# eudald-seeslab/mmsbm

Measured on NVIDIA B200. Metric: rating-updates/sec, higher is better.
Workload: dtype f64

## Files before the change

mmsbm_b200/build.py:

```python
import concurrent.futures as cf
import os
import subprocess
import sys

HERE = os.path.dirname(os.path.abspath(__file__))
CSRC = os.path.join(HERE, "csrc")
LIB = os.path.join(HERE, "libmmsbm_b200.so")
SOURCES = ["em_step.cu", "em_small.cu", "seg_inst_ch1.cu", "seg_inst_ch2.cu", "seg_inst_ch4.cu", "seg_inst_pair.cu", "seg_inst_hexa.cu", "graph_build.cu",
           "reductions.cu", "host_api.cu", "sharded_run.cu", "fold_in.cu"]
NVCC_FLAGS = [
    "-gencode", "arch=compute_100a,code=sm_100a", "-O3", "-lineinfo", "-std=c++17",
    "-Xcompiler", "-fPIC,-O3,-Wall", "-DMMSBM_B200",
]


def _nvcc():
    for cand in (os.environ.get("NVCC"), "/usr/local/cuda/bin/nvcc", "nvcc"):
        if cand and (os.path.isabs(cand) and os.path.exists(cand) or not os.path.isabs(cand)):
            return cand
    raise RuntimeError("nvcc not found")


def _stale(target, deps):
    if not os.path.exists(target):
        return True
    t = os.path.getmtime(target)
    return any(os.path.getmtime(d) > t for d in deps)


def build_library(force=False, verbose=False, check=False):
    nvcc = _nvcc()
    suffix, extra, lib = ("_chk.o", ["-DMMSBM_BOUNDS_CHECK"], LIB.replace(".so", "_check.so")) if check \
        else (".o", ["-DNDEBUG"], LIB)
    headers = [os.path.join(CSRC, "common.cuh"), os.path.join(CSRC, "segment_pass.cuh"), os.path.join(CSRC, "em_internal.cuh"),
               os.path.join(HERE, "..", "include", "mmsbm_b200.h"), os.path.abspath(__file__)]
    objs, jobs = [], []
    for src in SOURCES:
        s = os.path.join(CSRC, src)
        o = os.path.join(CSRC, src[:-3] + suffix)
        objs.append(o)
        if force or _stale(o, [s] + headers):
            cmd = [nvcc] + NVCC_FLAGS + extra + (["-Xptxas", "-v"] if verbose else []) + ["-c", s, "-o", o]
            jobs.append(cmd)
    if jobs:
        with cf.ThreadPoolExecutor(max_workers=len(jobs)) as ex:
            for cmd, res in zip(jobs, ex.map(lambda c: subprocess.run(c, capture_output=True, text=True), jobs)):
                if verbose or res.returncode:
                    sys.stderr.write(" ".join(cmd) + "\n" + res.stdout + res.stderr)
                if res.returncode:
                    raise RuntimeError("nvcc failed for " + cmd[-3])
    if jobs or force or _stale(lib, objs):
        cmd = [nvcc, "-shared", "-o", lib] + objs + ["-lcudart", "-ldl"]
        res = subprocess.run(cmd, capture_output=True, text=True)
        if res.returncode:
            sys.stderr.write(res.stdout + res.stderr)
            raise RuntimeError("link failed")
    return lib


if __name__ == "__main__":
    print(build_library(force="--force" in sys.argv, verbose="-v" in sys.argv, check="--check" in sys.argv))
```

mmsbm_b200/csrc/em_internal.cuh:

```cuda
#pragma once
#include "common.cuh"
#include "segment_pass.cuh"

namespace mmsbm {

constexpr int kPrSlabs = 128;

int env_int(const char* name, int dflt);
int sm_count();
void set_reserved_ctas(int n);

struct RunPlan { int hexas, pairs, pair_group0, single_from; };
RunPlan plan_runs(int NBp, int n_runs, bool hexa_table);

int launch_prep_p(const double* pr, int K, int L, int R, int ldk, int ldl, int n_runs, double* pw_u,
                  double* pn_u, double* pw_i, double* pn_i, cudaStream_t st);

int launch_interleave(const double* src, double* dst, int n_src, int n_dst, int row0, int ld,
                      int group0, int groups, int gs, cudaStream_t st);

int launch_w(const double* own, const double* pw, double* W, int M, int LD, int RNB, int n_runs,
             cudaStream_t st);
struct RowPublish {
  double* dst[3];
  int gs[3], group0[3], groups[3];
  int n_all, row0;
};
int launch_n(const double* G, const double* pn, const double* own, const int32_t* deg, double* out,
             int M, int LD, int RNB, int normalize, int n_runs, cudaStream_t st,
             const RowPublish* publish = nullptr);

int launch_segment_pass_and_fixup(SegArgs a, const double* nbr_pairs, const double* nbr_hexa,
                                  int64_t n_ratings, int n_runs, cudaStream_t st, bool no_long_segments = false);

int launch_pr(const double* own, const double* g, double* partial, const double* pr, double* pr_out,
              int nseg, int NA, int lda, int NBp, int K, int L, int R, int n_runs, bool transposed,
              bool normalize, cudaStream_t st);
int launch_finalize_pr(double* pr, int kl_total, int R, cudaStream_t st);

bool em_small_applicable(int64_t N, int R, int K, int L, int S);
size_t em_small_partial_elems(int R, int K);
int launch_em_small(const int32_t* useg, const int32_t* uadj, const int32_t* udeg, const int32_t* iseg,
                    const int32_t* iadj, const int32_t* ideg, const int32_t* usched, const int32_t* isched, int64_t N,
                    int U, int I, int R, int K, int L, int S, int iterations, double* theta_a, double* eta_a,
                    double* pr_a, double* theta_b, double* eta_b, double* pr_b, double* partial, size_t partial_elems,
                    cudaStream_t st);

}
```

mmsbm_b200/csrc/em_step.cu:

```cuda
#include <stdlib.h>

#include "common.cuh"
#include "em_internal.cuh"
#include "segment_pass.cuh"

namespace mmsbm {

constexpr int kPrThreads = 128;
constexpr int kPrBatch = 16;
constexpr int kGemmThreads = 256;
constexpr int kGemmBK = 32;
constexpr int kGemmTR = 4;

__global__ void __launch_bounds__(128) segment_fixup_kernel(const SegArgs A) {
  const int run = blockIdx.y, RNB = A.R * A.NBp;
  const int n_long = __ldg(A.sched + 2);
  const int32_t* long_seg = A.sched + 4 + 3 * A.pmax;
  const int32_t* long_slot0 = long_seg + A.lmax;
  for (int li = blockIdx.x; li < n_long; li += gridDim.x) {
    const int sg = __ldg(long_seg + li), s0 = __ldg(long_slot0 + li), s1 = __ldg(long_slot0 + li + 1);
    MMSBM_DEV_CHECK(sg >= 0 && sg < A.nseg && s0 >= 0 && s0 < s1 && s1 <= A.smax);
    const double* src = A.partial + ((size_t)run * A.smax + s0) * RNB;
    double* dst = A.wg + ((size_t)run * A.nseg + sg) * RNB;
    for (int o = threadIdx.x; o < RNB; o += blockDim.x) {
      double acc = 0.0;
      for (int k = 0; k < s1 - s0; ++k) acc += src[(size_t)k * RNB + o];
      dst[o] = acc;
    }
  }
}

__global__ void interleave_runs_kernel(const double* __restrict__ src, double* __restrict__ dst, int n_src,
                                       int n_dst, int row0, int ld, int group0, int groups, int gs) {
  const int c4 = ld >> 2;
  const size_t total = (size_t)groups * n_src * gs * c4;
  const size_t t = (size_t)blockIdx.x * blockDim.x + threadIdx.x;
  if (t >= total) return;
  const int c = (int)(t % c4);
  const int j = (int)((t / c4) % gs);
  const size_t rest = t / c4 / gs;
  const int id = (int)(rest % n_src);
  const size_t p = group0 + rest / n_src;
  const double4_t v = ldg256(src + (((size_t)(gs * p + j) * n_src + id) * ld + 4 * c));
  stg256(dst + (((p * n_dst + row0 + id) * gs + j) * ld + 4 * c), v);
}

__global__ void prep_p_kernel(const double* pr, int K, int L, int R, int ldk, int ldl, double* pw_u,
                              double* pn_u, double* pw_i, double* pn_i) {
  const int run = blockIdx.y;
  const int total = ldk * ldl * R;
  const int t = blockIdx.x * blockDim.x + threadIdx.x;
  if (t >= total) return;
  const int r = t % R, kl = t / R, lp = kl % ldl, kp = kl / ldl;
  double v = 0.0;
  if (kp < K && lp < L) v = __ldg(pr + (((size_t)run * K + kp) * L + lp) * R + r);
  const size_t base = (size_t)run * total;
  const int rnb_u = R * ldl, rnb_i = R * ldk;
  pw_u[base + (size_t)kp * rnb_u + r * ldl + lp] = v;
  pn_u[base + (size_t)(r * ldl + lp) * ldk + kp] = v;
  pw_i[base + (size_t)lp * rnb_i + r * ldk + kp] = v;
  pn_i[base + (size_t)(r * ldk + kp) * ldl + lp] = v;
}

struct GemmArgs {
  const double* A;
  const double* B;
  double* C;
  const double* own;
  const int32_t* deg;
  int M, N, Kd, lda, rg, normalize;
  int b_resident;
};

template <bool EPI>
__global__ void __launch_bounds__(kGemmThreads) small_gemm_kernel(const GemmArgs g) {
  constexpr int TR = kGemmTR;
  extern __shared__ __align__(32) unsigned char smem_raw[];
  const int BM = TR * g.rg, AS = kGemmBK + 2;
  double* Bs = reinterpret_cast<double*>(smem_raw);
  double* As = Bs + (size_t)(g.b_resident ? g.Kd : kGemmBK) * g.N;
  const int run = blockIdx.y;
  const int ncg = g.N >> 2, half = g.N >> 1;
  const int rgid = threadIdx.x / ncg, cg = threadIdx.x - rgid * ncg;
  const bool active = rgid < g.rg;
  const double* A = g.A + (size_t)run * g.M * g.lda;
  const double2* B2 = reinterpret_cast<const double2*>(g.B + (size_t)run * g.Kd * g.N);
  double2* Bs2 = reinterpret_cast<double2*>(Bs);
  if (g.b_resident)
    for (int t = threadIdx.x; t < (g.Kd * g.N) >> 1; t += kGemmThreads) Bs2[t] = __ldg(B2 + t);
  const int n_tiles = (g.M + BM - 1) / BM;
  for (int tile = blockIdx.x; tile < n_tiles; tile += gridDim.x) {
    const int row0 = tile * BM;
    double acc[TR][4];
#pragma unroll
    for (int i = 0; i < TR; ++i)
#pragma unroll
      for (int j = 0; j < 4; ++j) acc[i][j] = 0.0;

    for (int k0 = 0; k0 < g.Kd; k0 += kGemmBK) {
      const int bk = min(kGemmBK, g.Kd - k0);
      const int bk2 = bk >> 1;
      __syncthreads();
      for (int t = threadIdx.x; t < BM * bk2; t += kGemmThreads) {
        const int m = t / bk2, p2 = t - m * bk2;
        double2 v = make_double2(0.0, 0.0);
        if (row0 + m < g.M) v = __ldg(reinterpret_cast<const double2*>(A + (size_t)(row0 + m) * g.lda + k0) + p2);
        *reinterpret_cast<double2*>(As + m * AS + 2 * p2) = v;
      }
      if (!g.b_resident)
        for (int t = threadIdx.x; t < (bk * g.N) >> 1; t += kGemmThreads)
          Bs2[t] = __ldg(B2 + (((size_t)k0 * g.N) >> 1) + t);
      __syncthreads();
      if (active) {
        const double* ap = As + (size_t)(TR * rgid) * AS;
        const double* bp = Bs + (size_t)(g.b_resident ? k0 : 0) * g.N + 2 * cg;
        for (int kk = 0; kk < bk; kk += 2) {
          const double2 b00 = *reinterpret_cast<const double2*>(bp + (size_t)kk * g.N);
          const double2 b01 = *reinterpret_cast<const double2*>(bp + (size_t)kk * g.N + half);
          const double2 b10 = *reinterpret_cast<const double2*>(bp + (size_t)(kk + 1) * g.N);
          const double2 b11 = *reinterpret_cast<const double2*>(bp + (size_t)(kk + 1) * g.N + half);
#pragma unroll
          for (int i = 0; i < TR; ++i) {
            const double2 a = *reinterpret_cast<const double2*>(ap + i * AS + kk);
            acc[i][0] = fma(a.x, b00.x, acc[i][0]); acc[i][1] = fma(a.x, b00.y, acc[i][1]);
            acc[i][2] = fma(a.x, b01.x, acc[i][2]); acc[i][3] = fma(a.x, b01.y, acc[i][3]);
            acc[i][0] = fma(a.y, b10.x, acc[i][0]); acc[i][1] = fma(a.y, b10.y, acc[i][1]);
            acc[i][2] = fma(a.y, b11.x, acc[i][2]); acc[i][3] = fma(a.y, b11.y, acc[i][3]);
          }
        }
      }
    }
    if (active) {
#pragma unroll
      for (int i = 0; i < TR; ++i) {
        const int m = row0 + TR * rgid + i;
        if (m >= g.M) continue;
        const size_t off = ((size_t)run * g.M + m) * g.N + 2 * cg;
        double2 v0 = make_double2(acc[i][0], acc[i][1]), v1 = make_double2(acc[i][2], acc[i][3]);
        if (EPI) {
          const double2 o0 = __ldg(reinterpret_cast<const double2*>(g.own + off));
          const double2 o1 = __ldg(reinterpret_cast<const double2*>(g.own + off + half));
          v0.x *= o0.x; v0.y *= o0.y; v1.x *= o1.x; v1.y *= o1.y;
          if (g.normalize) {
            const double d = (double)max(__ldg(g.deg + m), 1);
            v0.x = v0.x / d; v0.y = v0.y / d; v1.x = v1.x / d; v1.y = v1.y / d;
          }
        }
        *reinterpret_cast<double2*>(g.C + off) = v0;
        *reinterpret_cast<double2*>(g.C + off + half) = v1;
      }
    }
  }
}

constexpr int kRowThreads = 256;

template <int LD, int ROWS>
__global__ void __launch_bounds__(kRowThreads) row_w_kernel(const double* __restrict__ own,
                                                            const double* __restrict__ pw,
                                                            double* __restrict__ W, int M, int RNB) {
  extern __shared__ __align__(32) unsigned char smem_raw[];
  double* Ps = reinterpret_cast<double*>(smem_raw);
  const int run = blockIdx.y;
  {
    const double2* src = reinterpret_cast<const double2*>(pw + (size_t)run * LD * RNB);
    double2* dst = reinterpret_cast<double2*>(Ps);
    for (int t = threadIdx.x; t < (LD * RNB) >> 1; t += kRowThreads) dst[t] = __ldg(src + t);
  }
  __syncthreads();
  const double* own_run = own + (size_t)run * M * LD;
  double* w_run = W + (size_t)run * M * RNB;
  for (int m0 = blockIdx.x * (kRowThreads * ROWS) + threadIdx.x; m0 < M; m0 += gridDim.x * (kRowThreads * ROWS)) {
    double o[ROWS][LD];
    int mr[ROWS];
#pragma unroll
    for (int j = 0; j < ROWS; ++j) {
      mr[j] = m0 + j * kRowThreads;
      const int mc = mr[j] < M ? mr[j] : m0;
#pragma unroll
      for (int c = 0; c < LD / 4; ++c) {
        const double4_t v = ldg256(own_run + (size_t)mc * LD + 4 * c);
        o[j][4 * c] = v.x; o[j][4 * c + 1] = v.y; o[j][4 * c + 2] = v.z; o[j][4 * c + 3] = v.w;
      }
    }
    for (int ob = 0; ob < RNB; ob += 4) {
      double4_t acc[ROWS];
#pragma unroll
      for (int j = 0; j < ROWS; ++j) acc[j] = double4_t{0.0, 0.0, 0.0, 0.0};
#pragma unroll
      for (int a = 0; a < LD; ++a) {
        const double4_t p = lds32(Ps + a * RNB + ob);
#pragma unroll
        for (int j = 0; j < ROWS; ++j) {
          acc[j].x = fma(o[j][a], p.x, acc[j].x); acc[j].y = fma(o[j][a], p.y, acc[j].y);
          acc[j].z = fma(o[j][a], p.z, acc[j].z); acc[j].w = fma(o[j][a], p.w, acc[j].w);
        }
      }
#pragma unroll
      for (int j = 0; j < ROWS; ++j)
        if (mr[j] < M) stg256(w_run + (size_t)mr[j] * RNB + ob, acc[j]);
    }
  }
}

template <int LD, int ROWS, int PF>
__global__ void __launch_bounds__(kRowThreads) row_n_kernel(const double* __restrict__ G,
                                                            const double* __restrict__ pn,
                                                            const double* __restrict__ own,
                                                            const int32_t* __restrict__ deg,
                                                            double* __restrict__ out, int M, int RNB,
                                                            int normalize, const RowPublish pub) {
  extern __shared__ __align__(32) unsigned char smem_raw[];
  double* Ps = reinterpret_cast<double*>(smem_raw);
  const int run = blockIdx.y;
  double* pdst = nullptr;
  int pgs = 1, pj = 0;
  size_t pgrp = 0;
#pragma unroll
  for (int t = 0; t < 3; ++t) {
    if (pub.dst[t] != nullptr && run >= pub.gs[t] * pub.group0[t] && run < pub.gs[t] * (pub.group0[t] + pub.groups[t])) {
      pdst = pub.dst[t]; pgs = pub.gs[t]; pgrp = (size_t)(run / pub.gs[t]); pj = run % pub.gs[t];
    }
  }
  {
    const double2* src = reinterpret_cast<const double2*>(pn + (size_t)run * LD * RNB);
    double2* dst = reinterpret_cast<double2*>(Ps);
    for (int t = threadIdx.x; t < (LD * RNB) >> 1; t += kRowThreads) dst[t] = __ldg(src + t);
  }
  __syncthreads();
  const double* g_run = G + (size_t)run * M * RNB;
  const double* own_run = own + (size_t)run * M * LD;
  double* out_run = out + (size_t)run * M * LD;
  for (int m0 = blockIdx.x * (kRowThreads * ROWS) + threadIdx.x; m0 < M; m0 += gridDim.x * (kRowThreads * ROWS)) {
    double acc[ROWS][LD];
    int mr[ROWS];
    const double* grow[ROWS];
#pragma unroll
    for (int j = 0; j < ROWS; ++j) {
      mr[j] = m0 + j * kRowThreads;
      grow[j] = g_run + (size_t)(mr[j] < M ? mr[j] : m0) * RNB;
#pragma unroll
      for (int a = 0; a < LD; ++a) acc[j][a] = 0.0;
    }
    for (int ob0 = 0; ob0 < RNB; ob0 += 4 * PF) {
      double4_t gq[ROWS][PF];
#pragma unroll
      for (int j = 0; j < ROWS; ++j)
#pragma unroll
        for (int p = 0; p < PF; ++p) gq[j][p] = ldg256(grow[j] + ob0 + 4 * p);
#pragma unroll
      for (int p = 0; p < PF; ++p) {
        const int ob = ob0 + 4 * p;
        double gv[ROWS][4];
#pragma unroll
        for (int j = 0; j < ROWS; ++j) {
          gv[j][0] = gq[j][p].x; gv[j][1] = gq[j][p].y; gv[j][2] = gq[j][p].z; gv[j][3] = gq[j][p].w;
        }
#pragma unroll
        for (int i = 0; i < 4; ++i) {
#pragma unroll
          for (int c = 0; c < LD / 4; ++c) {
            const double4_t pv = lds32(Ps + (ob + i) * LD + 4 * c);
#pragma unroll
            for (int j = 0; j < ROWS; ++j) {
              acc[j][4 * c] = fma(gv[j][i], pv.x, acc[j][4 * c]);         acc[j][4 * c + 1] = fma(gv[j][i], pv.y, acc[j][4 * c + 1]);
              acc[j][4 * c + 2] = fma(gv[j][i], pv.z, acc[j][4 * c + 2]); acc[j][4 * c + 3] = fma(gv[j][i], pv.w, acc[j][4 * c + 3]);
            }
          }
        }
      }
    }
#pragma unroll
    for (int j = 0; j < ROWS; ++j) {
      if (mr[j] >= M) continue;
      double d = 1.0;
      if (normalize) d = (double)max(__ldg(deg + mr[j]), 1);
#pragma unroll
      for (int c = 0; c < LD / 4; ++c) {
        const double4_t ov = ldg256(own_run + (size_t)mr[j] * LD + 4 * c);
        double4_t v{acc[j][4 * c] * ov.x, acc[j][4 * c + 1] * ov.y, acc[j][4 * c + 2] * ov.z, acc[j][4 * c + 3] * ov.w};
        if (normalize) { v.x = v.x / d; v.y = v.y / d; v.z = v.z / d; v.w = v.w / d; }
        stg256(out_run + (size_t)mr[j] * LD + 4 * c, v);
        if (pdst) stg256(pdst + (((pgrp * pub.n_all + pub.row0 + mr[j]) * pgs + pj) * LD + 4 * c), v);
      }
    }
  }
}

struct PrArgs {
  const double* own;
  const double* g;
  double* partial;
  int nseg, NA, lda, RNB;
};

__global__ void __launch_bounds__(kPrThreads) pr_accumulate_kernel(const PrArgs A) {
  extern __shared__ __align__(32) unsigned char smem_raw[];
  double* own_s = reinterpret_cast<double*>(smem_raw);
  double* g_s = own_s + kPrBatch * A.lda;
  const int run = blockIdx.y, slab = blockIdx.x;
  const int per = (A.nseg + kPrSlabs - 1) / kPrSlabs;
  const int s0 = slab * per, s1 = min(s0 + per, A.nseg);
  const int nout = A.NA * A.RNB;
  const int ta = A.lda >> 2, tb = A.RNB >> 2, n_tiles = ta * tb;
  const double* own_run = A.own + (size_t)run * A.nseg * A.lda;
  const double* g_run = A.g + (size_t)run * A.nseg * A.RNB;
  double* dst = A.partial + ((size_t)run * kPrSlabs + slab) * nout;

  for (int tile0 = 0; tile0 < n_tiles; tile0 += kPrThreads) {
    const int tile = tile0 + threadIdx.x;
    const bool on = tile < n_tiles;
    const int a0 = on ? 4 * (tile / tb) : 0, b0 = on ? 4 * (tile % tb) : 0;
    double acc[4][4];
#pragma unroll
    for (int i = 0; i < 4; ++i)
#pragma unroll
      for (int k = 0; k < 4; ++k) acc[i][k] = 0.0;
    for (int c0 = s0; c0 < s1; c0 += kPrBatch) {
      const int nb = min(kPrBatch, s1 - c0);
      __syncthreads();
      {
        const double2* src = reinterpret_cast<const double2*>(own_run + (size_t)c0 * A.lda);
        double2* d2 = reinterpret_cast<double2*>(own_s);
        for (int t = threadIdx.x; t < (nb * A.lda) >> 1; t += kPrThreads) d2[t] = __ldg(src + t);
        src = reinterpret_cast<const double2*>(g_run + (size_t)c0 * A.RNB);
        d2 = reinterpret_cast<double2*>(g_s);
        for (int t = threadIdx.x; t < (nb * A.RNB) >> 1; t += kPrThreads) d2[t] = __ldg(src + t);
      }
      __syncthreads();
      if (on) {
        for (int sg = 0; sg < nb; ++sg) {
          const double4_t o = lds32(own_s + sg * A.lda + a0);
          const double4_t g = lds32(g_s + sg * A.RNB + b0);
          const double ov[4] = {o.x, o.y, o.z, o.w};
#pragma unroll
          for (int i = 0; i < 4; ++i) {
            acc[i][0] = fma(ov[i], g.x, acc[i][0]); acc[i][1] = fma(ov[i], g.y, acc[i][1]);
            acc[i][2] = fma(ov[i], g.z, acc[i][2]); acc[i][3] = fma(ov[i], g.w, acc[i][3]);
          }
        }
      }
    }
    if (on) {
#pragma unroll
      for (int i = 0; i < 4; ++i)
        if (a0 + i < A.NA)
          stg256(dst + (size_t)(a0 + i) * A.RNB + b0, double4_t{acc[i][0], acc[i][1], acc[i][2], acc[i][3]});
    }
  }
}

struct PrFinArgs {
  const double* partial;
  const double* pr;
  double* pr_out;
  int K, L, R, NA, NBp, transposed, normalize;
};

constexpr int kFinWarps = 8;
__global__ void __launch_bounds__(kFinWarps * 32) pr_finalize_kernel(const PrFinArgs A) {
  extern __shared__ __align__(16) unsigned char smem_raw[];
  const int run = blockIdx.y, a = blockIdx.x;
  const int RNB = A.R * A.NBp, nout = A.NA * RNB;
  double* part_s = reinterpret_cast<double*>(smem_raw);
  double* tot_s = part_s + kFinWarps * RNB;
  const int lane = threadIdx.x & 31, warp = threadIdx.x >> 5;
  const double* part = A.partial + (size_t)run * kPrSlabs * nout + (size_t)a * RNB;
  constexpr int per = kPrSlabs / kFinWarps;
  for (int o = lane; o < RNB; o += 32) {
    double acc = 0.0;
#pragma unroll 4
    for (int s = warp * per; s < (warp + 1) * per; ++s) acc += part[(size_t)s * nout + o];
    part_s[warp * RNB + o] = acc;
  }
  __syncthreads();
  for (int o = threadIdx.x; o < RNB; o += blockDim.x) {
    double acc = 0.0;
    for (int w = 0; w < kFinWarps; ++w) acc += part_s[w * RNB + o];
    tot_s[o] = acc;
  }
  __syncthreads();
  const int NB = A.transposed ? A.K : A.L;
  for (int b = threadIdx.x; b < NB; b += blockDim.x) {
    const int k = A.transposed ? b : a, l = A.transposed ? a : b;
    const size_t kl = (size_t)k * A.L + l;
    const double* prs = A.pr + ((size_t)run * A.K * A.L + kl) * A.R;
    double* dst = A.pr_out + ((size_t)run * A.K * A.L + kl) * A.R;
    double tot = 0.0;
    for (int r = 0; r < A.R; ++r) {
      const double v = tot_s[r * A.NBp + b] * prs[r];
      dst[r] = v;
      tot += v;
    }
    if (A.normalize) {
      const double d = (tot == 0.0) ? 1.0 : tot;
      for (int r = 0; r < A.R; ++r) dst[r] = dst[r] / d;
    }
  }
}

__global__ void finalize_eta_kernel(double* eta, const int32_t* deg, int n_items, int ldl, int L,
                                    size_t total) {
  size_t t = (size_t)blockIdx.x * blockDim.x + threadIdx.x;
  if (t >= total) return;
  int col = (int)(t % ldl);
  size_t row = t / ldl;
  int item = (int)(row % n_items);
  if (col < L) eta[t] = eta[t] / (double)max(__ldg(deg + item), 1);
}

__global__ void finalize_pr_kernel(double* pr, int KL_total, int R) {
  int t = blockIdx.x * blockDim.x + threadIdx.x;
  if (t >= KL_total) return;
  double* row = pr + (size_t)t * R;
  double tot = 0.0;
  for (int r = 0; r < R; ++r) tot += row[r];
  const double d = (tot == 0.0) ? 1.0 : tot;
  for (int r = 0; r < R; ++r) row[r] = row[r] / d;
}

struct PassShape { int G, CH, UN, MINB; };

int env_int(const char* name, int dflt) {
  const char* v = getenv(name);
  return (v && *v) ? atoi(v) : dflt;
}

int sm_count() {
  static int cached[64] = {0};
  int dev = 0;
  if (cudaGetDevice(&dev) != cudaSuccess || dev < 0 || dev >= 64) return 148;
  if (cached[dev] == 0) {
    int n = 0;
    if (cudaDeviceGetAttribute(&n, cudaDevAttrMultiProcessorCount, dev) != cudaSuccess || n <= 0) n = 148;
    cached[dev] = n;
  }
  return cached[dev];
}

static PassShape choose_shape(int NBp, double avg_degree) {
  const int NCH = NBp / 4;
  int CH = 8;
  for (int c = 1; c <= 8; c *= 2) {
    if ((NCH + c - 1) / c <= 8) { CH = c; break; }
  }
  const int G = (NCH + CH - 1) / CH;
  PassShape sh{G, CH, 1, 1};
  (void)avg_degree;
  if (CH == 1) { sh.UN = (G == 1) ? 1 : (G == 2) ? 2 : 3; sh.MINB = 3; }
  else if (CH == 2) { sh.UN = 1; sh.MINB = 3; }
  return sh;
}

static int segs_per_cta_for(int64_t pmax, int64_t n_ratings, int grid_y) {
  const int e = env_int("MMSBM_SPC", 0);
  if (e > 0) return e;
  const double avg_piece = (double)(n_ratings > 0 ? n_ratings : 1) / (double)(pmax > 0 ? pmax : 1);
  int64_t spc = ((int64_t)(6144.0 / (avg_piece > 1.0 ? avg_piece : 1.0)) + kWarps / 2) / kWarps * kWarps;
  const int64_t fill = pmax * grid_y / (sm_count() * 3 * 6) / kWarps * kWarps;
  if (spc > fill) spc = fill;
  if (spc < kWarps) spc = kWarps;
  if (spc > 64) spc = 64;
  return (int)spc;
}

static bool pairs_enabled(int NBp, int n_runs) {
  return n_runs >= 2 && NBp <= 32 && env_int("MMSBM_PAIR", 1) != 0;
}

static int g_reserved_ctas = 0;
void set_reserved_ctas(int n) { g_reserved_ctas = n > 0 ? n : 0; }

static unsigned grid_x_for(const SegArgs& a, int ctas_per_sm) {
  if (!a.counters) return (unsigned)((a.pmax + a.segs_per_cta - 1) / a.segs_per_cta);
  int64_t resident = (int64_t)sm_count() * ctas_per_sm - g_reserved_ctas;
  if (resident < 1) resident = 1;
  const int64_t want = (a.pmax + kWarps - 1) / kWarps;
  return (unsigned)(want < resident ? want : resident);
}

static bool hexa_enabled(int NBp, int n_runs) {
  return n_runs >= 6 && NBp == 20 && env_int("MMSBM_HEXA", 1) != 0;
}

RunPlan plan_runs(int NBp, int n_runs, bool hexa_table) {
  RunPlan p{0, 0, 0, 0};
  if (hexa_table && hexa_enabled(NBp, n_runs)) p.hexas = n_runs / 6;
  p.single_from = 6 * p.hexas;
  if (pairs_enabled(NBp, n_runs - p.single_from)) {
    p.pairs = (n_runs - p.single_from) / 2;
    p.pair_group0 = p.single_from / 2;
    p.single_from += 2 * p.pairs;
  }
  return p;
}

static int launch_segment_pass_impl(SegArgs a, const double* nbr_pairs, const double* nbr_hexa,
                                    int64_t n_ratings, int n_runs, cudaStream_t st) {
  const double avg_degree = (double)n_ratings / (double)a.nseg;
  PassShape sh = choose_shape(a.NBp, avg_degree);
  const int un_e = env_int("MMSBM_UN", 0), occ_e = env_int("MMSBM_OCC", 0);
  const RunPlan plan = plan_runs(a.NBp, n_runs, nbr_hexa != nullptr);
  const int single_from = plan.single_from;
  if (plan.hexas > 0) {
    const int hexas = plan.hexas;
    SegArgs p = a;
    p.nbr = nbr_hexa;
    p.run_base = 0;
    p.grp_base = 0;
    p.segs_per_cta = segs_per_cta_for(a.pmax, n_ratings, hexas);
    const unsigned gx = grid_x_for(p, occ_e > 0 ? occ_e : 3);
    if (p.counters) a.counters += hexas;
    const size_t smem = seg_smem_bytes(p, 6);
    MMSBM_REQUIRE(smem <= 227 * 1024, MMSBM_ERANGE, "segment pass needs %zu bytes of shared memory", smem);
    int rc = MMSBM_ERANGE;
    if (un_e > 0 || occ_e > 0)
      rc = launch_segment_pass_hexa(p, sh.G, un_e > 0 ? un_e : 3, occ_e > 0 ? occ_e : 3, dim3(gx, hexas), smem, st);
    if (rc == MMSBM_ERANGE) rc = launch_segment_pass_hexa(p, sh.G, 3, 3, dim3(gx, hexas), smem, st);
    if (rc) {
      if (rc == MMSBM_ERANGE) set_error("no six-run segment-pass variant for G=%d", sh.G);
      return rc;
    }
    if (single_from == n_runs && plan.pairs == 0) return 0;
  }
  if (plan.pairs > 0) {
    MMSBM_REQUIRE(nbr_pairs, MMSBM_EINVAL, "segment pass: the table of run pairs is missing");
    const int pairs = plan.pairs;
    SegArgs p = a;
    p.nbr = nbr_pairs;
    p.run_base = 6 * plan.hexas;
    p.grp_base = plan.pair_group0;
    p.counters = a.counters;
    p.segs_per_cta = segs_per_cta_for(a.pmax, n_ratings, pairs);
    const unsigned gx = grid_x_for(p, occ_e > 0 ? occ_e : 3);
    if (p.counters) a.counters += pairs;
    const size_t smem = seg_smem_bytes(p, 2);
    MMSBM_REQUIRE(smem <= 227 * 1024, MMSBM_ERANGE, "segment pass needs %zu bytes of shared memory", smem);
    int UN = (sh.G == 1) ? 2 : 3, MINB = 3;
    int rc = MMSBM_ERANGE;
    if (un_e > 0 || occ_e > 0)
      rc = launch_segment_pass_pair(p, sh.G, un_e > 0 ? un_e : UN, occ_e > 0 ? occ_e : MINB, dim3(gx, pairs), smem, st);
    if (rc == MMSBM_ERANGE) rc = launch_segment_pass_pair(p, sh.G, UN, MINB, dim3(gx, pairs), smem, st);
    if (rc == MMSBM_ERANGE && sh.G == 1) rc = launch_segment_pass_pair(p, sh.G, 2, 3, dim3(gx, pairs), smem, st);
    if (rc) {
      if (rc == MMSBM_ERANGE) set_error("no paired segment-pass variant for G=%d", sh.G);
      return rc;
    }
  }
  if (single_from == n_runs) return 0;
  a.run_base = single_from;
  a.segs_per_cta = segs_per_cta_for(a.pmax, n_ratings, n_runs - single_from);
  const unsigned gx = grid_x_for(a, occ_e > 0 ? occ_e : sh.MINB);
  const dim3 grid(gx, n_runs - single_from);
  const size_t smem = seg_smem_bytes(a, 1);
  MMSBM_REQUIRE(smem <= 227 * 1024, MMSBM_ERANGE,
                "segment pass needs %zu bytes of shared memory (R=%d, row stride %d)", smem, a.R, a.NBp);
  auto go = [&](const PassShape& p) {
    switch (p.CH) {
      case 1: return launch_segment_pass_ch1(a, p.G, p.UN, p.MINB, grid, smem, st);
      case 2: return launch_segment_pass_ch2(a, p.G, p.UN, p.MINB, grid, smem, st);
      case 4: return launch_segment_pass_ch4(a, p.G, p.UN, p.MINB, grid, smem, st);
      default: return launch_segment_pass_ch8(a, p.G, p.UN, p.MINB, grid, smem, st);
    }
  };
  if (un_e > 0 || occ_e > 0) {
    PassShape alt = sh;
    if (un_e > 0) alt.UN = un_e;
    if (occ_e > 0) alt.MINB = occ_e;
    const int rc = go(alt);
    if (rc != MMSBM_ERANGE) return rc;
  }
  const int rc = go(sh);
  if (rc == MMSBM_ERANGE) set_error("no segment-pass variant for G=%d CH=%d UN=%d", sh.G, sh.CH, sh.UN);
  return rc;
}

int launch_segment_pass_and_fixup(SegArgs a, const double* nbr_pairs, const double* nbr_hexa,
                                  int64_t n_ratings, int n_runs, cudaStream_t st, bool no_long_segments) {
  int rc = launch_segment_pass_impl(a, nbr_pairs, nbr_hexa, n_ratings, n_runs, st);
  if (rc) return rc;
  if (no_long_segments) return 0;
  const int64_t fix_ctas = 4 * sm_count();
  const unsigned gx = (unsigned)(a.lmax < fix_ctas ? a.lmax : fix_ctas);
  segment_fixup_kernel<<<dim3(gx, n_runs), 128, 0, st>>>(a);
  MMSBM_LAUNCH_CHECK("segment_fixup_kernel");
  return 0;
}

template <bool EPI>
static int launch_gemm(GemmArgs g, int n_runs, cudaStream_t st) {
  const int ncg = g.N / 4;
  MMSBM_REQUIRE(g.N % 4 == 0 && g.Kd % 4 == 0 && ncg >= 1 && ncg <= kGemmThreads, MMSBM_ERANGE,
                "small gemm: N=%d Kd=%d not supported (N <= 1024, multiples of 4)", g.N, g.Kd);
  int rg = kGemmThreads / ncg;
  if (rg > 32) rg = 32;
  g.rg = rg;
  const int BM = kGemmTR * rg;
  size_t smem = ((size_t)g.Kd * g.N + (size_t)BM * (kGemmBK + 2)) * 8;
  g.b_resident = smem <= 200 * 1024;
  if (!g.b_resident) smem = ((size_t)kGemmBK * g.N + (size_t)BM * (kGemmBK + 2)) * 8;
  MMSBM_REQUIRE(smem <= 227 * 1024, MMSBM_ERANGE,
                "small gemm needs %zu bytes of shared memory (K*L*R too large)", smem);
  auto kern = small_gemm_kernel<EPI>;
  MMSBM_CUDA(cudaFuncSetAttribute(kern, cudaFuncAttributeMaxDynamicSharedMemorySize, (int)smem));
  const int n_tiles = (g.M + BM - 1) / BM;
  int per_run = (sm_count() * 3 + n_runs - 1) / n_runs;
  if (per_run > n_tiles) per_run = n_tiles;
  if (per_run < 1) per_run = 1;
  kern<<<dim3(per_run, n_runs), kGemmThreads, smem, st>>>(g);
  MMSBM_LAUNCH_CHECK("small_gemm_kernel");
  return 0;
}

int launch_w(const double* own, const double* pw, double* W, int M, int LD, int RNB, int n_runs,
             cudaStream_t st) {
  const size_t smem = (size_t)LD * RNB * 8;
  const int rows_env = env_int("MMSBM_ROWS", 2);
#define MMSBM_ROW_W(LDv)                                                                        \
  if (LD == LDv && smem <= 200 * 1024) {                                                        \
    constexpr int kRows = (LDv <= 24) ? 2 : 1;             \
    const bool two = kRows == 2 && rows_env == 2;                                               \
    auto kern = two ? row_w_kernel<LDv, kRows> : row_w_kernel<LDv, 1>;                          \
    const int per = kRowThreads * (two ? 2 : 1);                                                \
    const int gx = min((M + per - 1) / per, sm_count() * 2);                                           \
    MMSBM_CUDA(cudaFuncSetAttribute(kern, cudaFuncAttributeMaxDynamicSharedMemorySize, (int)smem)); \
    kern<<<dim3(gx, n_runs), kRowThreads, smem, st>>>(own, pw, W, M, RNB);                      \
    MMSBM_LAUNCH_CHECK("row_w_kernel");                                                         \
    return 0;                                                                                   \
  }
  MMSBM_ROW_W(4) MMSBM_ROW_W(8) MMSBM_ROW_W(12) MMSBM_ROW_W(16) MMSBM_ROW_W(20) MMSBM_ROW_W(24)
  MMSBM_ROW_W(28) MMSBM_ROW_W(32)
#undef MMSBM_ROW_W
  GemmArgs g{own, pw, W, nullptr, nullptr, M, RNB, LD, LD, 0, 0, 0};
  return launch_gemm<false>(g, n_runs, st);
}

int launch_n(const double* G, const double* pn, const double* own, const int32_t* deg, double* out,
             int M, int LD, int RNB, int normalize, int n_runs, cudaStream_t st, const RowPublish* publish) {
  const size_t smem = (size_t)LD * RNB * 8;
  RowPublish pub{};
  if (publish) pub = *publish;
  const int rows_env = env_int("MMSBM_ROWS_N", 1);
  int pf = env_int("MMSBM_ROWN_PF", 5);
  if (pf != 1 && pf != 2 && pf != 5) pf = 1;
  if ((RNB / 4) % pf != 0) pf = ((RNB / 4) % 2 == 0 && pf != 1) ? 2 : 1;
#define MMSBM_ROW_N_GO(kern, two)                                                               \
  {                                                                                             \
    const int per = kRowThreads * ((two) ? 2 : 1);                                              \
    const int gx = min((M + per - 1) / per, sm_count() * 2);                                    \
    MMSBM_CUDA(cudaFuncSetAttribute(kern, cudaFuncAttributeMaxDynamicSharedMemorySize, (int)smem)); \
    kern<<<dim3(gx, n_runs), kRowThreads, smem, st>>>(G, pn, own, deg, out, M, RNB, normalize, pub); \
    MMSBM_LAUNCH_CHECK("row_n_kernel");                                                         \
    return 0;                                                                                   \
  }
#define MMSBM_ROW_N(LDv)                                                                        \
  if (LD == LDv && smem <= 200 * 1024) {                                                        \
    constexpr int kRows = (LDv <= 24) ? 2 : 1;         \
    const bool two = kRows == 2 && rows_env == 2;                                               \
    if (two) MMSBM_ROW_N_GO((row_n_kernel<LDv, kRows, 1>), true)                                \
    if (pf == 5) MMSBM_ROW_N_GO((row_n_kernel<LDv, 1, 5>), false)                               \
    if (pf == 2) MMSBM_ROW_N_GO((row_n_kernel<LDv, 1, 2>), false)                               \
    MMSBM_ROW_N_GO((row_n_kernel<LDv, 1, 1>), false)                                            \
  }
  MMSBM_ROW_N(4) MMSBM_ROW_N(8) MMSBM_ROW_N(12) MMSBM_ROW_N(16) MMSBM_ROW_N(20) MMSBM_ROW_N(24)
  MMSBM_ROW_N(28) MMSBM_ROW_N(32)
#undef MMSBM_ROW_N_GO
#undef MMSBM_ROW_N
  MMSBM_REQUIRE(!publish, MMSBM_ERANGE, "row publishing needs row strides of at most 32 doubles");
  GemmArgs g{G, pn, out, own, deg, M, LD, RNB, RNB, 0, normalize, 0};
  return launch_gemm<true>(g, n_runs, st);
}

int launch_prep_p(const double* pr, int K, int L, int R, int ldk, int ldl, int n_runs, double* pw_u,
                  double* pn_u, double* pw_i, double* pn_i, cudaStream_t st) {
  const int total = ldk * ldl * R;
  prep_p_kernel<<<dim3((total + 255) / 256, n_runs), 256, 0, st>>>(pr, K, L, R, ldk, ldl, pw_u, pn_u, pw_i, pn_i);
  MMSBM_LAUNCH_CHECK("prep_p_kernel");
  return 0;
}

int launch_interleave(const double* src, double* dst, int n_src, int n_dst, int row0, int ld, int group0,
                      int groups, int gs, cudaStream_t st) {
  const size_t tot = (size_t)groups * n_src * gs * (ld / 4);
  if (tot == 0) return 0;
  interleave_runs_kernel<<<(unsigned)((tot + 255) / 256), 256, 0, st>>>(src, dst, n_src, n_dst, row0, ld,
                                                                        group0, groups, gs);
  MMSBM_LAUNCH_CHECK("interleave_runs_kernel");
  return 0;
}

int launch_pr(const double* own, const double* g, double* partial, const double* pr, double* pr_out,
              int nseg, int NA, int lda, int NBp, int K, int L, int R, int n_runs, bool transposed,
              bool normalize, cudaStream_t st) {
  PrArgs pa{};
  pa.own = own; pa.g = g; pa.partial = partial;
  pa.nseg = nseg; pa.NA = NA; pa.lda = lda; pa.RNB = R * NBp;
  const size_t smem = (size_t)kPrBatch * (pa.lda + pa.RNB) * 8;
  MMSBM_CUDA(cudaFuncSetAttribute(pr_accumulate_kernel, cudaFuncAttributeMaxDynamicSharedMemorySize,
                                  (int)smem));
  pr_accumulate_kernel<<<dim3(kPrSlabs, n_runs), kPrThreads, smem, st>>>(pa);
  MMSBM_LAUNCH_CHECK("pr_accumulate_kernel");
  PrFinArgs fa{};
  fa.partial = partial; fa.pr = pr; fa.pr_out = pr_out;
  fa.K = K; fa.L = L; fa.R = R; fa.NA = NA; fa.NBp = NBp;
  fa.transposed = transposed ? 1 : 0;
  fa.normalize = normalize ? 1 : 0;
  const size_t fin_smem = (size_t)(kFinWarps + 1) * R * NBp * 8;
  MMSBM_CUDA(cudaFuncSetAttribute(pr_finalize_kernel, cudaFuncAttributeMaxDynamicSharedMemorySize, (int)fin_smem));
  pr_finalize_kernel<<<dim3(NA, n_runs), kFinWarps * 32, fin_smem, st>>>(fa);
  MMSBM_LAUNCH_CHECK("pr_finalize_kernel");
  return 0;
}

int launch_finalize_pr(double* pr, int kl_total, int R, cudaStream_t st) {
  finalize_pr_kernel<<<(kl_total + 127) / 128, 128, 0, st>>>(pr, kl_total, R);
  MMSBM_LAUNCH_CHECK("finalize_pr_kernel");
  return 0;
}

struct EmDims {
  int U, I, R, K, L, S, ldk, ldl, rnb_u, rnb_i;
  bool emit_items;
  int nseg_e, NA_e, NBp_e;
  size_t p_elems, wg_u_elems, wg_i_elems, partial_elems, slots_u_elems, slots_i_elems;
  size_t th2_elems, et2_elems;
  size_t et6_elems;
  size_t ctr_elems;
  int64_t lmax, smax, pmax_u, pmax_i;
};

static EmDims em_dims(int64_t N, int U, int I, int R, int K, int L, int S) {
  EmDims d;
  d.U = U; d.I = I; d.R = R; d.K = K; d.L = L; d.S = S;
  d.ldk = row_stride(K); d.ldl = row_stride(L);
  d.rnb_u = R * d.ldl; d.rnb_i = R * d.ldk;
  d.emit_items = (I <= U);
  d.nseg_e = d.emit_items ? I : U;
  d.NA_e = d.emit_items ? L : K;
  d.NBp_e = d.emit_items ? d.ldk : d.ldl;
  d.p_elems = (size_t)S * d.ldk * d.ldl * R;
  d.wg_u_elems = (size_t)S * U * d.rnb_u;
  d.wg_i_elems = (size_t)S * I * d.rnb_i;
  d.partial_elems = (size_t)S * kPrSlabs * d.NA_e * R * d.NBp_e;
  d.lmax = N / MMSBM_PIECE_LEN + 1;
  d.smax = 2 * (N / MMSBM_PIECE_LEN) + 1;
  d.pmax_u = (int64_t)U + N / MMSBM_PIECE_LEN + 1;
  d.pmax_i = (int64_t)I + N / MMSBM_PIECE_LEN + 1;
  d.slots_u_elems = (size_t)S * d.smax * d.rnb_u;
  d.slots_i_elems = (size_t)S * d.smax * d.rnb_i;
  d.th2_elems = (size_t)(S / 2) * 2 * U * d.ldk;
  d.et2_elems = (size_t)(S / 2) * 2 * I * d.ldl;
  d.et6_elems = (size_t)(S / 6) * 6 * I * d.ldl;
  d.ctr_elems = 2 * ((size_t)S + 8);
  return d;
}

static size_t em_main_bytes(const EmDims& d) {
  return 4 * align_up(d.p_elems * 8) + align_up(d.wg_u_elems * 8) + align_up(d.wg_i_elems * 8) +
         align_up(d.partial_elems * 8) + align_up(d.slots_u_elems * 8) + align_up(d.slots_i_elems * 8) +
         align_up(d.th2_elems * 8) + align_up(d.et2_elems * 8) + align_up(d.et6_elems * 8) + align_up(d.ctr_elems * 4) + 256;
}

}

using namespace mmsbm;

extern "C" int mmsbm_em_workspace_bytes(int64_t N, int32_t U, int32_t I, int32_t R, int32_t K,
                                        int32_t L, int32_t S, size_t* bytes) {
  MMSBM_REQUIRE(bytes && N >= 0 && U > 0 && I > 0 && R > 0 && K > 0 && L > 0 && S > 0, MMSBM_EINVAL,
                "mmsbm_em_workspace_bytes: bad argument");
  EmDims d = em_dims(N, U, I, R, K, L, S);
  *bytes = em_main_bytes(d);
  if (em_small_applicable(N, R, K, L, S)) *bytes += align_up(em_small_partial_elems(R, K) * 8);
  return 0;
}

struct Overlap {
  bool no_long_u = false, no_long_i = false;
  cudaStream_t side = nullptr;
  cudaEvent_t e[6] = {nullptr, nullptr, nullptr, nullptr, nullptr, nullptr};
  bool two_branch = false;
};

static int em_step_impl(const int32_t* useg, const int32_t* uadj, const int32_t* udeg,
                        const int32_t* iseg, const int32_t* iadj, const int32_t* ideg,
                        const int32_t* usched, const int32_t* isched, int64_t N, int32_t U, int32_t I, int32_t R, int32_t K, int32_t L,
                        int32_t S, const double* theta, const double* eta, const double* pr,
                        double* theta_out, double* eta_out, double* pr_out, int32_t flags,
                        void* ws, size_t ws_bytes, void* stream, cudaEvent_t* ev,
                        const Overlap* ov = nullptr) {
  MMSBM_REQUIRE(useg && uadj && udeg && iseg && iadj && ideg && usched && isched && theta && eta && pr &&
                    theta_out && eta_out && pr_out && ws, MMSBM_EINVAL, "mmsbm_em_step: null pointer");
  MMSBM_REQUIRE(N >= 0 && U > 0 && I > 0 && R > 0 && K > 0 && L > 0 && S > 0, MMSBM_EINVAL,
                "mmsbm_em_step: bad size");
  MMSBM_REQUIRE(K <= 256 && L <= 256 && R <= 31, MMSBM_ERANGE,
                "mmsbm_em_step: K, L <= 256 and R <= 31 supported (K=%d L=%d R=%d)", K, L, R);
  cudaStream_t st = static_cast<cudaStream_t>(stream);
  EmDims d = em_dims(N, U, I, R, K, L, S);
  Arena arena(ws, ws_bytes);
  double* pw_u = arena.take<double>(d.p_elems);
  double* pn_u = arena.take<double>(d.p_elems);
  double* pw_i = arena.take<double>(d.p_elems);
  double* pn_i = arena.take<double>(d.p_elems);
  double* wg_u = arena.take<double>(d.wg_u_elems);
  double* wg_i = arena.take<double>(d.wg_i_elems);
  double* partial = arena.take<double>(d.partial_elems);
  double* slots_u = arena.take<double>(d.slots_u_elems);
  double* slots_i = arena.take<double>(d.slots_i_elems);
  double* th2 = arena.take<double>(d.th2_elems);
  double* et2 = arena.take<double>(d.et2_elems);
  double* et6 = arena.take<double>(d.et6_elems);
  int32_t* counters = arena.take<int32_t>(d.ctr_elems);
  MMSBM_REQUIRE(pw_u && pn_u && pw_i && pn_i && wg_u && wg_i && partial && slots_u && slots_i && th2 && et2 && et6 && counters,
                MMSBM_ENOMEM,
                "mmsbm_em_step: workspace too small (%zu)", ws_bytes);
  int rc;
  const bool dyn = env_int("MMSBM_DYN", N >= ((int64_t)1 << 22) ? 1 : 0) != 0;
#define MMSBM_MARK(k) do { if (ev) MMSBM_CUDA(cudaEventRecord(ev[k], st)); } while (0)
  MMSBM_MARK(0);
  cudaStream_t s2 = ov ? ov->side : st;
#define MMSBM_FORK(k) do { if (ov) { MMSBM_CUDA(cudaEventRecord(ov->e[k], st)); \
                                     MMSBM_CUDA(cudaStreamWaitEvent(s2, ov->e[k], 0)); } } while (0)
#define MMSBM_JOIN(k) do { if (ov) { MMSBM_CUDA(cudaEventRecord(ov->e[k], s2)); \
                                     MMSBM_CUDA(cudaStreamWaitEvent(st, ov->e[k], 0)); } } while (0)
#define MMSBM_SIDE_DONE(k) do { if (ov) MMSBM_CUDA(cudaEventRecord(ov->e[k], s2)); } while (0)
  if (ov && ov->two_branch) {
    if (dyn) MMSBM_CUDA(cudaMemsetAsync(counters, 0, d.ctr_elems * 4, st));
    if ((rc = launch_prep_p(pr, K, L, R, d.ldk, d.ldl, S, pw_u, pn_u, pw_i, pn_i, st))) return rc;
    MMSBM_FORK(0);
    auto pr_step = [&](cudaStream_t s) {
      return launch_pr(d.emit_items ? eta : theta, d.emit_items ? wg_i : wg_u, partial, pr, pr_out, d.nseg_e,
                       d.NA_e, d.emit_items ? d.ldl : d.ldk, d.NBp_e, K, L, R, S, d.emit_items,
                       (flags & MMSBM_RAW_ETA_PR) == 0, s);
    };
    if (hexa_enabled(d.ldl, S) && (rc = launch_interleave(eta, et6, I, I, 0, d.ldl, 0, S / 6, 6, st))) return rc;
    if (pairs_enabled(d.ldl, S) && (rc = launch_interleave(eta, et2, I, I, 0, d.ldl, 0, S / 2, 2, st))) return rc;
    if ((rc = launch_w(theta, pw_u, wg_u, U, d.ldk, d.rnb_u, S, st))) return rc;
    {
      SegArgs a{useg, uadj, usched, eta, wg_u, slots_u, d.pmax_u, d.lmax, d.smax, U, I, d.ldl, R, 0, 0, 0,
                dyn ? counters : nullptr};
      if ((rc = launch_segment_pass_and_fixup(a, et2, et6, N, S, st, ov->no_long_u))) return rc;
    }
    if ((rc = launch_n(wg_u, pn_u, theta, udeg, theta_out, U, d.ldk, d.rnb_u,
                       (flags & MMSBM_RAW_THETA) ? 0 : 1, S, st))) return rc;
    if (!d.emit_items && (rc = pr_step(st))) return rc;
    if (pairs_enabled(d.ldk, S) && (rc = launch_interleave(theta, th2, U, U, 0, d.ldk, 0, S / 2, 2, s2))) return rc;
    if ((rc = launch_w(eta, pw_i, wg_i, I, d.ldl, d.rnb_i, S, s2))) return rc;
    {
      SegArgs a{iseg, iadj, isched, theta, wg_i, slots_i, d.pmax_i, d.lmax, d.smax, I, U, d.ldk, R, 0, 0, 0,
                dyn ? counters + d.ctr_elems / 2 : nullptr};
      if ((rc = launch_segment_pass_and_fixup(a, th2, nullptr, N, S, s2, ov->no_long_i))) return rc;
    }
    if ((rc = launch_n(wg_i, pn_i, eta, ideg, eta_out, I, d.ldl, d.rnb_i,
                       (flags & MMSBM_RAW_ETA_PR) ? 0 : 1, S, s2))) return rc;
    if (d.emit_items && (rc = pr_step(s2))) return rc;
    MMSBM_JOIN(1);
    return 0;
  }
  {
    if (dyn) MMSBM_CUDA(cudaMemsetAsync(counters, 0, d.ctr_elems * 4, st));
    if ((rc = launch_prep_p(pr, K, L, R, d.ldk, d.ldl, S, pw_u, pn_u, pw_i, pn_i, st))) return rc;
    MMSBM_FORK(0);
    if (hexa_enabled(d.ldl, S) && (rc = launch_interleave(eta, et6, I, I, 0, d.ldl, 0, S / 6, 6, st))) return rc;
    if (pairs_enabled(d.ldl, S) && (rc = launch_interleave(eta, et2, I, I, 0, d.ldl, 0, S / 2, 2, st))) return rc;
    if (pairs_enabled(d.ldk, S) && (rc = launch_interleave(theta, th2, U, U, 0, d.ldk, 0, S / 2, 2, st))) return rc;
    if ((rc = launch_w(theta, pw_u, wg_u, U, d.ldk, d.rnb_u, S, st))) return rc;
    if ((rc = launch_w(eta, pw_i, wg_i, I, d.ldl, d.rnb_i, S, s2))) return rc;
    MMSBM_SIDE_DONE(1);
  }
  MMSBM_MARK(1);
  {
    SegArgs a{useg, uadj, usched, eta, wg_u, slots_u, d.pmax_u, d.lmax, d.smax, U, I, d.ldl, R, 0, 0, 0,
              dyn ? counters : nullptr};
    if ((rc = launch_segment_pass_and_fixup(a, et2, et6, N, S, st, ov && ov->no_long_u))) return rc;
  }
  MMSBM_MARK(2);
  MMSBM_FORK(2);
  if ((rc = launch_n(wg_u, pn_u, theta, udeg, theta_out, U, d.ldk, d.rnb_u,
                     (flags & MMSBM_RAW_THETA) ? 0 : 1, S, s2))) return rc;
  MMSBM_SIDE_DONE(4);
  MMSBM_MARK(3);
  if (ov) MMSBM_CUDA(cudaStreamWaitEvent(st, ov->e[1], 0));
  {
    SegArgs a{iseg, iadj, isched, theta, wg_i, slots_i, d.pmax_i, d.lmax, d.smax, I, U, d.ldk, R, 0, 0, 0,
              dyn ? counters + d.ctr_elems / 2 : nullptr};
    if ((rc = launch_segment_pass_and_fixup(a, th2, nullptr, N, S, st, ov && ov->no_long_i))) return rc;
  }
  MMSBM_MARK(4);
  MMSBM_FORK(3);
  if ((rc = launch_n(wg_i, pn_i, eta, ideg, eta_out, I, d.ldl, d.rnb_i,
                     (flags & MMSBM_RAW_ETA_PR) ? 0 : 1, S, s2))) return rc;
  MMSBM_SIDE_DONE(5);
  MMSBM_MARK(5);
  if ((rc = launch_pr(d.emit_items ? eta : theta, d.emit_items ? wg_i : wg_u, partial, pr, pr_out, d.nseg_e,
                      d.NA_e, d.emit_items ? d.ldl : d.ldk, d.NBp_e, K, L, R, S, d.emit_items,
                      (flags & MMSBM_RAW_ETA_PR) == 0, st))) return rc;
  MMSBM_MARK(6);
  MMSBM_MARK(7);
  if (ov) {
    MMSBM_CUDA(cudaStreamWaitEvent(st, ov->e[4], 0));
    MMSBM_CUDA(cudaStreamWaitEvent(st, ov->e[5], 0));
  }
#undef MMSBM_MARK
#undef MMSBM_FORK
#undef MMSBM_JOIN
#undef MMSBM_SIDE_DONE
  return 0;
}

extern "C" int mmsbm_em_step(const int32_t* useg, const int32_t* uadj, const int32_t* udeg,
                             const int32_t* iseg, const int32_t* iadj, const int32_t* ideg, const int32_t* usched,
                 const int32_t* isched,
                             int64_t N, int32_t U, int32_t I, int32_t R, int32_t K, int32_t L,
                             int32_t S, const double* theta, const double* eta, const double* pr,
                             double* theta_out, double* eta_out, double* pr_out, int32_t flags,
                             void* ws, size_t ws_bytes, void* stream) {
  return em_step_impl(useg, uadj, udeg, iseg, iadj, ideg, usched, isched, N, U, I, R, K, L, S, theta, eta, pr,
                      theta_out, eta_out, pr_out, flags, ws, ws_bytes, stream, nullptr);
}

extern "C" int mmsbm_em_step_profiled(const int32_t* useg, const int32_t* uadj, const int32_t* udeg,
                                      const int32_t* iseg, const int32_t* iadj, const int32_t* ideg, const int32_t* usched,
                 const int32_t* isched,
                                      int64_t N, int32_t U, int32_t I, int32_t R, int32_t K,
                                      int32_t L, int32_t S, const double* theta, const double* eta,
                                      const double* pr, double* theta_out, double* eta_out,
                                      double* pr_out, int32_t flags, void* ws, size_t ws_bytes,
                                      void* stream, float* ms7) {
  MMSBM_REQUIRE(ms7, MMSBM_EINVAL, "mmsbm_em_step_profiled: null output");
  cudaEvent_t ev[8];
  for (int k = 0; k < 8; ++k) MMSBM_CUDA(cudaEventCreate(&ev[k]));
  int rc = em_step_impl(useg, uadj, udeg, iseg, iadj, ideg, usched, isched, N, U, I, R, K, L, S, theta, eta, pr,
                        theta_out, eta_out, pr_out, flags, ws, ws_bytes, stream, ev);
  if (rc == 0) {
    cudaError_t e = cudaEventSynchronize(ev[7]);
    if (e != cudaSuccess) { set_error("cudaEventSynchronize: %s", cudaGetErrorString(e)); rc = (int)e; }
    for (int k = 0; k < 7 && rc == 0; ++k) cudaEventElapsedTime(&ms7[k], ev[k], ev[k + 1]);
  }
  for (int k = 0; k < 8; ++k) cudaEventDestroy(ev[k]);
  return rc;
}

extern "C" int mmsbm_em_run(const int32_t* useg, const int32_t* uadj, const int32_t* udeg,
                            const int32_t* iseg, const int32_t* iadj, const int32_t* ideg, const int32_t* usched,
                 const int32_t* isched,
                            int64_t N, int32_t U, int32_t I, int32_t R, int32_t K, int32_t L,
                            int32_t S, int32_t iterations, double* theta_a, double* eta_a,
                            double* pr_a, double* theta_b, double* eta_b, double* pr_b, void* ws,
                            size_t ws_bytes, void* stream) {
  MMSBM_REQUIRE(iterations >= 0, MMSBM_EINVAL, "mmsbm_em_run: negative iteration count");
  cudaStream_t st = static_cast<cudaStream_t>(stream);
  if (iterations > 0 && N >= 0 && U > 0 && I > 0 && R > 0 && K > 0 && L > 0 && em_small_applicable(N, R, K, L, S) &&
      useg && uadj && udeg && iseg && iadj && ideg && usched && isched && theta_a && eta_a && pr_a && theta_b &&
      eta_b && pr_b && ws) {
    const size_t main_bytes = em_main_bytes(em_dims(N, U, I, R, K, L, S));
    const size_t part_elems = em_small_partial_elems(R, K);
    if (ws_bytes >= main_bytes + part_elems * 8) {
      const int rc = launch_em_small(useg, uadj, udeg, iseg, iadj, ideg, usched, isched, N, U, I, R, K, L, S,
                                     iterations, theta_a, eta_a, pr_a, theta_b, eta_b, pr_b,
                                     reinterpret_cast<double*>(static_cast<char*>(ws) + main_bytes), part_elems, st);
      if (rc != MMSBM_ERANGE) return rc;
    }
  }
  Overlap ov;
  const bool small = (double)N * S < 5.0e7;
  const bool overlap = iterations > 0 && getenv("MMSBM_NO_OVERLAP") == nullptr;
  if (overlap) {
    MMSBM_CUDA(cudaStreamCreateWithFlags(&ov.side, cudaStreamNonBlocking));
    for (auto& e : ov.e) MMSBM_CUDA(cudaEventCreateWithFlags(&e, cudaEventDisableTiming));
    ov.two_branch = small && getenv("MMSBM_FORCE_OVERLAP") == nullptr;
  }
  {
    cudaStreamCaptureStatus cs0 = cudaStreamCaptureStatusNone;
    if (small && iterations >= 8 && cudaStreamIsCapturing(st, &cs0) == cudaSuccess && cs0 == cudaStreamCaptureStatusNone) {
      int32_t hu[4] = {0, 0, 1, 0}, hi[4] = {0, 0, 1, 0};
      MMSBM_CUDA(cudaMemcpyAsync(hu, usched, sizeof(hu), cudaMemcpyDeviceToHost, st));
      MMSBM_CUDA(cudaMemcpyAsync(hi, isched, sizeof(hi), cudaMemcpyDeviceToHost, st));
      MMSBM_CUDA(cudaStreamSynchronize(st));
      ov.no_long_u = hu[2] == 0;
      ov.no_long_i = hi[2] == 0;
    }
  }
  auto step = [&](bool fwd) {
    return em_step_impl(useg, uadj, udeg, iseg, iadj, ideg, usched, isched, N, U, I, R, K, L, S,
                        fwd ? theta_a : theta_b, fwd ? eta_a : eta_b, fwd ? pr_a : pr_b,
                        fwd ? theta_b : theta_a, fwd ? eta_b : eta_a, fwd ? pr_b : pr_a, 0, ws,
                        ws_bytes, stream, nullptr, overlap ? &ov : nullptr);
  };
  struct Cleanup {
    Overlap& o;
    ~Cleanup() {
      for (auto& e : o.e) if (e) cudaEventDestroy(e);
      if (o.side) cudaStreamDestroy(o.side);
    }
  } cleanup{ov};
  int done = 0;
  cudaStreamCaptureStatus cap = cudaStreamCaptureStatusNone;
  if (small && getenv("MMSBM_NO_GRAPH") == nullptr && iterations >= 8 && st != nullptr && cudaStreamIsCapturing(st, &cap) == cudaSuccess &&
      cap == cudaStreamCaptureStatusNone) {
    int rc = step(true);
    if (rc == 0) rc = step(false);
    if (rc) return rc;
    done = 2;
    cudaGraph_t graph = nullptr;
    cudaGraphExec_t exec = nullptr;
    const int64_t l0 = mmsbm_launch_count();
    MMSBM_CUDA(cudaStreamBeginCapture(st, cudaStreamCaptureModeThreadLocal));
    rc = step(true);
    if (rc == 0) rc = step(false);
    cudaError_t e = cudaStreamEndCapture(st, &graph);
    const int per_pair = (int)(mmsbm_launch_count() - l0);
    count_launch(-per_pair);
    if (rc == 0 && e == cudaSuccess && graph) e = cudaGraphInstantiate(&exec, graph, 0);
    if (graph) cudaGraphDestroy(graph);
    if (rc) return rc;
    if (e == cudaSuccess && exec) {
      for (; done + 2 <= iterations; done += 2) {
        MMSBM_CUDA(cudaGraphLaunch(exec, st));
        count_launch(per_pair);
      }
      cudaGraphExecDestroy(exec);
    } else {
      (void)cudaGetLastError();
    }
  }
  for (int it = done; it < iterations; ++it) {
    int rc = step((it & 1) == 0);
    if (rc) return rc;
  }
  return 0;
}

extern "C" int mmsbm_em_finalize(double* eta, const int32_t* ideg, int32_t I, int32_t L, double* pr,
                                 int32_t K, int32_t R, int32_t S, void* stream) {
  MMSBM_REQUIRE(eta && ideg && pr && I > 0 && L > 0 && K > 0 && R > 0 && S > 0, MMSBM_EINVAL,
                "mmsbm_em_finalize: bad argument");
  cudaStream_t st = static_cast<cudaStream_t>(stream);
  const int ldl = row_stride(L);
  size_t total = (size_t)S * I * ldl;
  finalize_eta_kernel<<<(unsigned)((total + 255) / 256), 256, 0, st>>>(eta, ideg, I, ldl, L, total);
  MMSBM_LAUNCH_CHECK("finalize_eta_kernel");
  return launch_finalize_pr(pr, S * K * L, R, st);
}
```

mmsbm_b200/csrc/segment_pass.cuh:

```cuda
#pragma once
#include <type_traits>

#include "common.cuh"

namespace mmsbm {

constexpr int kWarps = 8;

struct alignas(16) double4_t { double x, y, z, w; };

__device__ __forceinline__ double4_t ldg256(const double* p) {
  double4_t v;
  asm("ld.global.nc.v4.f64 {%0,%1,%2,%3}, [%4];"
      : "=d"(v.x), "=d"(v.y), "=d"(v.z), "=d"(v.w) : "l"(p));
  return v;
}
__device__ __forceinline__ void stg256(double* p, const double4_t& v) {
  asm volatile("st.global.v4.f64 [%0], {%1,%2,%3,%4};" ::"l"(p), "d"(v.x), "d"(v.y), "d"(v.z), "d"(v.w)
               : "memory");
}
__device__ __forceinline__ double4_t lds32(const double* p) {
  const double2 a = *reinterpret_cast<const double2*>(p);
  const double2 b = *reinterpret_cast<const double2*>(p + 2);
  return double4_t{a.x, a.y, b.x, b.y};
}
__device__ __forceinline__ void cp_async16(void* smem_dst, const void* gmem_src) {
  asm volatile("cp.async.cg.shared.global [%0], [%1], 16;" ::"r"(
                   (uint32_t)__cvta_generic_to_shared(smem_dst)), "l"(gmem_src) : "memory");
}
__device__ __forceinline__ void cp_async_commit() { asm volatile("cp.async.commit_group;" ::: "memory"); }
template <int N>
__device__ __forceinline__ void cp_async_wait() { asm volatile("cp.async.wait_group %0;" ::"n"(N) : "memory"); }

__device__ __forceinline__ double rcp_clamped(double x) {
  x = (x < kEps) ? kEps : x;
  double r;
  asm("rcp.approx.ftz.f64 %0, %1;" : "=d"(r) : "d"(x));
  const double e = fma(-x, r, 1.0);
  const double t = fma(e, e, e);
  return fma(r, t, r);
}

struct SegArgs {
  const int32_t* seg;
  const int32_t* adj;
  const int32_t* sched;
  const double* nbr;
  double* wg;
  double* partial;
  int64_t pmax, lmax, smax;
  int nseg, nnbr, NBp, R, segs_per_cta;
  int run_base;
  int grp_base;
  int* counters;
};

__host__ __device__ constexpr int w_buffers(int runs) { return runs > 2 ? 1 : 2; }
inline size_t seg_smem_bytes(const SegArgs& a, int runs) {
  return (size_t)kWarps * w_buffers(runs) * runs * a.R * a.NBp * 8 + 32;
}

template <int G>
struct GroupSum {
  int s1, s2, s4, s6;
  int lead, r1, r2, r3;
  bool is0, is1, is2, is3, is14, is03;
  __device__ __forceinline__ GroupSum(int leader, int q) {
    s1 = (leader + (q + 1) % G) & 31;
    s2 = (leader + (q + 2) % G) & 31;
    s4 = (leader + (q + 4) % G) & 31;
    s6 = (leader + (q + 6) % G) & 31;
    lead = leader & 31;
    is0 = q == 0; is1 = q == 1; is2 = q == 2; is3 = q == 3; is14 = (q == 1) | (q == 4); is03 = (q == 0) | (q == 3);
    r1 = (leader + (q == 0 ? 1 : q == 1 ? 2 : q == 2 ? 0 : q == 3 ? 4 : 3)) & 31;
    r2 = (leader + (q == 0 ? 2 : q == 1 ? 4 : q == 2 ? 3 : q == 3 ? 3 : 0)) & 31;
    r3 = (leader + (q == 0 ? 3 : q == 1 ? 4 : q == 2 ? 1 : q)) & 31;
  }
  __device__ __forceinline__ double sum3(double a0, double a1, double a2) const {
    static_assert(G == 5, "sum3 is the 5-lane schedule");
    const double pub = is0 ? a2 : (is14 ? a0 : a1);
    const double tgt = is03 ? a0 : (is2 ? a2 : a1);
    const double t = tgt + __shfl_sync(kFull, pub, r1);
    const double vo = is0 ? a1 : (is2 ? a0 : a2);
    double u = is1 ? a2 : t;
    const double v = is1 ? t : vo;
    const double x2 = __shfl_sync(kFull, v, r2);
    u += is3 ? 0.0 : x2;
    const double x3 = __shfl_sync(kFull, u, r3);
    return (is1 ? v : u) + x3;
  }
  __device__ __forceinline__ double from_lane(double x, int j) const { return __shfl_sync(kFull, x, lead + j); }
  __device__ __forceinline__ double operator()(double p) const {
    if constexpr (G == 1) {
      return p;
    } else if constexpr (G == 2) {
      return p + __shfl_xor_sync(kFull, p, 1);
    } else if constexpr (G == 4) {
      p += __shfl_xor_sync(kFull, p, 1);
      return p + __shfl_xor_sync(kFull, p, 2);
    } else if constexpr (G == 8) {
      p += __shfl_xor_sync(kFull, p, 1);
      p += __shfl_xor_sync(kFull, p, 2);
      return p + __shfl_xor_sync(kFull, p, 4);
    } else if constexpr (G == 3) {
      const double w2 = p + __shfl_sync(kFull, p, s1);
      return w2 + __shfl_sync(kFull, p, s2);
    } else if constexpr (G == 5) {
      const double w2 = p + __shfl_sync(kFull, p, s1);
      const double w4 = w2 + __shfl_sync(kFull, w2, s2);
      return w4 + __shfl_sync(kFull, p, s4);
    } else if constexpr (G == 6) {
      const double w2 = p + __shfl_sync(kFull, p, s1);
      const double w4 = w2 + __shfl_sync(kFull, w2, s2);
      return w4 + __shfl_sync(kFull, w2, s4);
    } else {
      static_assert(G == 7, "groups have 1..8 lanes");
      const double w2 = p + __shfl_sync(kFull, p, s1);
      const double w4 = w2 + __shfl_sync(kFull, w2, s2);
      const double w6 = w4 + __shfl_sync(kFull, w2, s4);
      return w6 + __shfl_sync(kFull, p, s6);
    }
  }
};

template <int G, int CH, int UN, int MINB, int RUNS>
__global__ void __launch_bounds__(kWarps * 32, MINB)
segment_pass_kernel(const SegArgs A) {
  constexpr int GR = G * RUNS;
  constexpr int RPS = 32 / GR;
  constexpr int SLOTS = UN * RPS;
  static_assert(SLOTS <= 32, "a chunk's ids must fit one coalesced 32-lane load");
  extern __shared__ __align__(32) unsigned char smem_raw[];
  const int lane = threadIdx.x & 31, warp = threadIdx.x >> 5;
  const int R = A.R, NBp = (CH == 1) ? 4 * G : A.NBp, RNB = R * NBp;
  const int NCH = NBp >> 2;

  constexpr int WB = w_buffers(RUNS);
  double* wbuf = reinterpret_cast<double*>(smem_raw) + (size_t)warp * WB * RUNS * RNB;
  int* ctr = reinterpret_cast<int*>(smem_raw + (size_t)kWarps * WB * RUNS * RNB * 8);
  if (threadIdx.x == 0) *ctr = 0;
  __syncthreads();

  const int grp = lane / GR, lig = lane - grp * GR;
  const int rsel = lig / G, q = lig - rsel * G;
  const bool lane_on = grp < RPS;
  const int run0 = A.run_base + blockIdx.y * RUNS, run = run0 + rsel;
  const int32_t* piece_seg = A.sched + 4;
  const int32_t* piece_idx = piece_seg + A.pmax;
  const int32_t* piece_slot = piece_idx + A.pmax;
  const int n_pieces = __ldg(A.sched);
  const bool dyn = A.counters != nullptr;
  int* claim = dyn ? A.counters + blockIdx.y : ctr;
  const int seg_lo = dyn ? 0 : blockIdx.x * A.segs_per_cta;
  const int seg_hi = dyn ? n_pieces : min(seg_lo + A.segs_per_cta, n_pieces);
  const int first = dyn ? blockIdx.x * kWarps + warp : seg_lo + warp;
  const int claim_base = dyn ? gridDim.x * kWarps : seg_lo + kWarps;
  const double* nbr_run = (RUNS == 1) ? A.nbr + (size_t)run * A.nnbr * NBp
                                      : A.nbr + ((size_t)(A.grp_base + blockIdx.y) * A.nnbr * RUNS + rsel) * NBp;
  int coff[CH];
  bool con[CH];
#pragma unroll
  for (int c = 0; c < CH; ++c) {
    const int chunk = c * G + q;
    con[c] = lane_on && chunk < NCH;
    coff[c] = con[c] ? 4 * chunk : 0;
  }
  const GroupSum<G> group_sum(grp * GR + rsel * G, q);

  auto fetch_w = [&](int s_, int b_) {
#pragma unroll 1
    for (int r2 = 0; r2 < RUNS; ++r2) {
      const double* src = A.wg + ((size_t)(run0 + r2) * A.nseg + s_) * RNB;
      double* dst = wbuf + (size_t)(b_ * RUNS + r2) * RNB;
#pragma unroll 1
      for (int p = lane; p < (RNB >> 1); p += 32) cp_async16(dst + 2 * p, src + 2 * p);
    }
  };

  int pi = first, buf = 0;
  int sg = 0, pinfo_pref = 0, bend_pref = 0;
  auto prefetch_piece = [&](int p_, int b_, int& sg_out) {
    MMSBM_DEV_CHECK(p_ >= 0 && p_ < A.pmax);
    sg_out = __ldg(piece_seg + p_);
    MMSBM_DEV_CHECK(sg_out >= 0 && sg_out < A.nseg);
    pinfo_pref = (lane == 0) ? __ldg(piece_idx + p_) : (lane == 1) ? __ldg(piece_slot + p_) : 0;
    if (lane <= R) bend_pref = __ldg(A.seg + (size_t)sg_out * R + lane);
    if constexpr (WB == 2) fetch_w(sg_out, b_);
  };
  if (pi < seg_hi) prefetch_piece(pi, 0, sg);
  cp_async_commit();

  while (pi < seg_hi) {
    const int bend_reg = bend_pref, pinfo = pinfo_pref;
    int t = 0;
    if (lane == 0) t = atomicAdd(claim, 1);
    const int pi_next = claim_base + __shfl_sync(kFull, t, 0);
    int sg_next = 0;
    if (pi_next < seg_hi) prefetch_piece(pi_next, buf ^ 1, sg_next);
    cp_async_commit();
    const int slot = __shfl_sync(kFull, pinfo, 1);
    const int beg = __shfl_sync(kFull, bend_reg, 0) + __shfl_sync(kFull, pinfo, 0) * MMSBM_PIECE_LEN;
    const int end = min(beg + MMSBM_PIECE_LEN, __shfl_sync(kFull, bend_reg, R));
    MMSBM_DEV_CHECK(slot >= -1 && slot < A.smax && beg >= 0 && beg <= end);
    int cur_ids = 0;
    if (lane < SLOTS && beg + lane < end) cur_ids = ld_stream(A.adj + beg + lane);
    if constexpr (WB == 2) {
      cp_async_wait<1>();
    } else {
      fetch_w(sg, 0);
      cp_async_commit();
      cp_async_wait<0>();
    }
    __syncwarp();
    const double* wb = wbuf + (size_t)((WB == 2 ? buf : 0) * RUNS + rsel) * RNB;
    double* gout = (slot < 0) ? A.wg + ((size_t)run * A.nseg + sg) * RNB
                              : A.partial + ((size_t)run * A.smax + slot) * RNB;

    double4_t g[CH], wr[CH];
    auto flush = [&](int r, bool any) {
#pragma unroll
      for (int c = 0; c < CH; ++c) {
        double4_t v = g[c];
        if (any) {
#pragma unroll
          for (int off = 16; off > 0; off >>= 1) {
            if (off < RPS) {
              const double tx = __shfl_down_sync(kFull, v.x, off * GR);
              const double ty = __shfl_down_sync(kFull, v.y, off * GR);
              const double tz = __shfl_down_sync(kFull, v.z, off * GR);
              const double tw = __shfl_down_sync(kFull, v.w, off * GR);
              if (grp + off < RPS) { v.x += tx; v.y += ty; v.z += tz; v.w += tw; }
            }
          }
        }
        if (grp == 0 && con[c]) stg256(gout + r * NBp + coff[c], v);
      }
    };

    int lo = beg;
    for (int r = 0; r < R; ++r) {
      const int le = min(end, __shfl_sync(kFull, bend_reg, r + 1));
#pragma unroll
      for (int c = 0; c < CH; ++c) g[c] = double4_t{0.0, 0.0, 0.0, 0.0};
      const bool any = lo < le;
      if (any) {
#pragma unroll
        for (int c = 0; c < CH; ++c)
          wr[c] = con[c] ? lds32(wb + r * NBp + coff[c]) : double4_t{0.0, 0.0, 0.0, 0.0};
        for (int base = lo; base < le; base += SLOTS) {
          const int cnt = min(SLOTS, le - base);
          auto chunk = [&](auto ns_tag) {
            constexpr int NS = decltype(ns_tag)::value;
            double4_t x[NS][CH];
#pragma unroll
            for (int un = 0; un < NS; ++un) {
              const int sl = un * RPS + grp;
              int id = __shfl_sync(kFull, cur_ids, sl & 31);
              if (sl >= cnt) id = 0;
              MMSBM_DEV_CHECK(id >= 0 && id < A.nnbr);
              const double* row = nbr_run + (size_t)id * (RUNS * NBp);
#pragma unroll
              for (int c = 0; c < CH; ++c) x[un][c] = ldg256(row + coff[c]);
            }
            {
              const int nxt = base + cnt + lane;
              cur_ids = (lane < SLOTS && nxt < end) ? ld_stream(A.adj + nxt) : 0;
            }
            double im[NS];
#pragma unroll
            for (int un = 0; un < NS; ++un) {
              double part = 0.0, part2 = 0.0;
#pragma unroll
              for (int c = 0; c < CH; ++c) {
                part = fma(x[un][c].x, wr[c].x, part); part2 = fma(x[un][c].y, wr[c].y, part2);
                part = fma(x[un][c].z, wr[c].z, part); part2 = fma(x[un][c].w, wr[c].w, part2);
              }
              im[un] = part + part2;
            }
            if constexpr (G == 5 && NS == 3) {
              const double mine = rcp_clamped(group_sum.sum3(im[0], im[1], im[2]));
#pragma unroll
              for (int un = 0; un < NS; ++un) {
                im[un] = group_sum.from_lane(mine, un);
                if (un * RPS + grp >= cnt) im[un] = 0.0;
              }
            } else {
#pragma unroll
              for (int un = 0; un < NS; ++un) {
                im[un] = rcp_clamped(group_sum(im[un]));
                if (un * RPS + grp >= cnt) im[un] = 0.0;
              }
            }
#pragma unroll
            for (int un = 0; un < NS; ++un) {
#pragma unroll
              for (int c = 0; c < CH; ++c) {
                g[c].x = fma(x[un][c].x, im[un], g[c].x); g[c].y = fma(x[un][c].y, im[un], g[c].y);
                g[c].z = fma(x[un][c].z, im[un], g[c].z); g[c].w = fma(x[un][c].w, im[un], g[c].w);
              }
            }
          };
          static_assert(UN <= 6, "extend the step-count dispatch");
          const int ns = (cnt + RPS - 1) / RPS;
          if (ns == UN) chunk(std::integral_constant<int, UN>{});
          else if (ns == 1) chunk(std::integral_constant<int, 1>{});
          else if (UN > 2 && ns == 2) chunk(std::integral_constant<int, (UN > 2 ? 2 : 1)>{});
          else if (UN > 3 && ns == 3) chunk(std::integral_constant<int, (UN > 3 ? 3 : 1)>{});
          else if (UN > 4 && ns == 4) chunk(std::integral_constant<int, (UN > 4 ? 4 : 1)>{});
          else if (UN > 5 && ns == 5) chunk(std::integral_constant<int, (UN > 5 ? 5 : 1)>{});
        }
        lo = le;
      }
      flush(r, any);
    }
    __syncwarp();
    buf ^= 1;
    sg = sg_next;
    pi = pi_next;
  }
  cp_async_wait<0>();
}

int launch_segment_pass_ch1(const SegArgs& a, int G, int UN, int MINB, dim3 grid, size_t smem, cudaStream_t st);
int launch_segment_pass_pair(const SegArgs& a, int G, int UN, int MINB, dim3 grid, size_t smem, cudaStream_t st);
int launch_segment_pass_hexa(const SegArgs& a, int G, int UN, int MINB, dim3 grid, size_t smem, cudaStream_t st);
int launch_segment_pass_ch2(const SegArgs& a, int G, int UN, int MINB, dim3 grid, size_t smem, cudaStream_t st);
int launch_segment_pass_ch4(const SegArgs& a, int G, int UN, int MINB, dim3 grid, size_t smem, cudaStream_t st);
int launch_segment_pass_ch8(const SegArgs& a, int G, int UN, int MINB, dim3 grid, size_t smem, cudaStream_t st);

#define MMSBM_SEG_LAUNCH(Gv, CHv, UNv, MBv) MMSBM_SEG_LAUNCH_R(Gv, CHv, UNv, MBv, 1)
#define MMSBM_SEG_LAUNCH_R(Gv, CHv, UNv, MBv, RUNSv)                                           \
  if (G == Gv && UN == UNv && MINB == MBv) {                                                   \
    auto kern = segment_pass_kernel<Gv, CHv, UNv, MBv, RUNSv>;                                 \
    MMSBM_CUDA(cudaFuncSetAttribute(kern, cudaFuncAttributeMaxDynamicSharedMemorySize, (int)smem)); \
    kern<<<grid, dim3(kWarps * 32), smem, st>>>(a);                                            \
    MMSBM_LAUNCH_CHECK("segment_pass_kernel");                                                 \
    return 0;                                                                                  \
  }

}
```

mmsbm_b200/csrc/sharded_run.cu:

```cuda
#include <dlfcn.h>
#include <nccl.h>

#include <chrono>
#include <stdlib.h>
#include <string.h>

#include "common.cuh"
#include "em_internal.cuh"

namespace mmsbm {

struct NcclApi {
  void* handle = nullptr;
  ncclResult_t (*GetUniqueId)(ncclUniqueId*) = nullptr;
  ncclResult_t (*CommInitRank)(ncclComm_t*, int, ncclUniqueId, int) = nullptr;
  ncclResult_t (*CommDestroy)(ncclComm_t) = nullptr;
  ncclResult_t (*AllReduce)(const void*, void*, size_t, ncclDataType_t, ncclRedOp_t, ncclComm_t, cudaStream_t) = nullptr;
  const char* (*GetErrorString)(ncclResult_t) = nullptr;
};
static NcclApi g_nccl;

#define MMSBM_NCCL(expr)                                                                   \
  do {                                                                                     \
    ncclResult_t r__ = (expr);                                                             \
    if (r__ != ncclSuccess) {                                                              \
      set_error("%s failed: %s", #expr, g_nccl.GetErrorString ? g_nccl.GetErrorString(r__) : "?"); \
      return 1000 + (int)r__;                                                              \
    }                                                                                      \
  } while (0)

static int nccl_ready() {
  MMSBM_REQUIRE(g_nccl.handle, MMSBM_EINVAL, "NCCL is not loaded: call mmsbm_nccl_load first");
  return 0;
}

struct Table { size_t off; int gs, group0, groups, ld, n_all; };
struct GridLayout {
  Table eta[3], theta[2];
  size_t half_bytes, total_bytes;
};

static GridLayout grid_layout(int U, int I, int K, int L, int S) {
  const int ldk = row_stride(K), ldl = row_stride(L);
  const RunPlan pu = plan_runs(ldl, S, true), pi = plan_runs(ldk, S, false);
  GridLayout g{};
  size_t off = 0;
  auto put = [&](Table& t, int gs, int group0, int groups, int ld, int n_all, int addr_groups) {
    t = Table{off, gs, group0, groups, ld, n_all};
    off += align_up((size_t)addr_groups * gs * n_all * ld * 8);
  };
  put(g.eta[0], 6, 0, pu.hexas, ldl, I, pu.hexas);
  put(g.eta[1], 2, pu.pair_group0, pu.pairs, ldl, I, pu.pairs ? S / 2 : 0);
  put(g.eta[2], 1, pu.single_from, S - pu.single_from, ldl, I, S > pu.single_from ? S : 0);
  put(g.theta[0], 2, pi.pair_group0, pi.pairs, ldk, U, pi.pairs ? S / 2 : 0);
  put(g.theta[1], 1, pi.single_from, S - pi.single_from, ldk, U, S > pi.single_from ? S : 0);
  g.half_bytes = off;
  g.total_bytes = 2 * off + 256;
  return g;
}

static RowPublish row_publish(const void* base, const GridLayout& g, const Table* tabs, int n_tabs, int half,
                              int n_all, int row0) {
  RowPublish p{};
  for (int k = 0; k < n_tabs && k < 3; ++k) {
    const Table& t = tabs[k];
    if (t.groups == 0) continue;
    p.dst[k] = reinterpret_cast<double*>(const_cast<char*>(static_cast<const char*>(base)) +
                                         (size_t)half * g.half_bytes + t.off);
    p.gs[k] = t.gs; p.group0[k] = t.group0; p.groups[k] = t.groups;
  }
  p.n_all = n_all; p.row0 = row0;
  return p;
}

static const double* table_ptr(const void* base, const GridLayout& g, int half, const Table& t) {
  if (t.groups == 0) return nullptr;
  return reinterpret_cast<const double*>(static_cast<const char*>(base) + (size_t)half * g.half_bytes + t.off);
}

struct Exchange {
  int peers = 0;
  cudaStream_t side = nullptr;
  cudaStream_t aux = nullptr;
  cudaEvent_t p_ready = nullptr, w2_ready = nullptr, pass1_done = nullptr, aux_done = nullptr;
  cudaStream_t cp[16] = {nullptr};
  cudaEvent_t ready = nullptr;
  cudaEvent_t done[16] = {nullptr};
  cudaEvent_t partial = nullptr, pr_done = nullptr;
  cudaEvent_t arrived[2][2] = {{nullptr, nullptr}, {nullptr, nullptr}};
  int open(int world) {
    peers = world - 1;
    if (peers <= 0) return 0;
    MMSBM_REQUIRE(peers <= 16, MMSBM_ERANGE, "sharded runs support up to 17 ranks");
    MMSBM_CUDA(cudaStreamCreateWithFlags(&side, cudaStreamNonBlocking));
    {
      int lo = 0, hi = 0;
      MMSBM_CUDA(cudaDeviceGetStreamPriorityRange(&lo, &hi));
      MMSBM_CUDA(cudaStreamCreateWithPriority(&aux, cudaStreamNonBlocking, hi));
    }
    for (int p = 0; p < peers; ++p) {
      MMSBM_CUDA(cudaStreamCreateWithFlags(&cp[p], cudaStreamNonBlocking));
      MMSBM_CUDA(cudaEventCreateWithFlags(&done[p], cudaEventDisableTiming));
    }
    cudaEvent_t* evs[] = {&ready, &partial, &pr_done, &arrived[0][0], &arrived[0][1], &arrived[1][0], &arrived[1][1],
                          &p_ready, &w2_ready, &pass1_done, &aux_done};
    for (cudaEvent_t* e : evs) MMSBM_CUDA(cudaEventCreateWithFlags(e, cudaEventDisableTiming));
    return 0;
  }
  ~Exchange() {
    cudaEvent_t evs[] = {ready, partial, pr_done, arrived[0][0], arrived[0][1], arrived[1][0], arrived[1][1],
                         p_ready, w2_ready, pass1_done, aux_done};
    for (cudaEvent_t e : evs) if (e) cudaEventDestroy(e);
    for (int p = 0; p < peers; ++p) {
      if (done[p]) cudaEventDestroy(done[p]);
      if (cp[p]) cudaStreamDestroy(cp[p]);
    }
    if (side) cudaStreamDestroy(side);
    if (aux) cudaStreamDestroy(aux);
  }
};

static int publish_side(const mmsbm_shard_t& sh, const GridLayout& g, const Table* tabs, int n_tabs,
                        const double* own_rows, int n_own, int lo, int half, cudaStream_t st,
                        const Exchange& ex) {
  char* mine = static_cast<char*>(sh.exchange_dev[sh.rank]);
  for (int k = 0; k < n_tabs && own_rows; ++k) {
    const Table& t = tabs[k];
    if (t.groups == 0) continue;
    double* dst = reinterpret_cast<double*>(mine + (size_t)half * g.half_bytes + t.off);
    int rc = launch_interleave(own_rows, dst, n_own, t.n_all, lo, t.ld, t.group0, t.groups, t.gs, st);
    if (rc) return rc;
  }
  if (sh.world == 1) return 0;
  MMSBM_CUDA(cudaEventRecord(ex.ready, st));
  for (int d = 1; d < sh.world; ++d) {
    const int peer = (sh.rank + d) % sh.world;
    cudaStream_t cs = ex.cp[d - 1];
    char* theirs = static_cast<char*>(sh.exchange_dev[peer]);
    MMSBM_CUDA(cudaStreamWaitEvent(cs, ex.ready, 0));
    for (int k = 0; k < n_tabs; ++k) {
      const Table& t = tabs[k];
      if (t.groups == 0) continue;
      const size_t row_bytes = (size_t)t.gs * t.ld * 8;
      const size_t pitch = (size_t)t.n_all * row_bytes;
      const size_t o = (size_t)half * g.half_bytes + t.off + ((size_t)t.group0 * t.n_all + lo) * row_bytes;
      MMSBM_CUDA(cudaMemcpy2DAsync(theirs + o, pitch, mine + o, pitch, (size_t)n_own * row_bytes,
                                   (size_t)t.groups, cudaMemcpyDeviceToDevice, cs));
    }
    MMSBM_CUDA(cudaEventRecord(ex.done[d - 1], cs));
  }
  return 0;
}

static int barrier_on_side(const mmsbm_shard_t& sh, const GridLayout& g, const Exchange& ex, cudaEvent_t signal) {
  for (int p = 0; p < ex.peers; ++p) MMSBM_CUDA(cudaStreamWaitEvent(ex.side, ex.done[p], 0));
  double* scratch = reinterpret_cast<double*>(static_cast<char*>(sh.exchange_dev[sh.rank]) + 2 * g.half_bytes);
  MMSBM_NCCL(g_nccl.AllReduce(scratch, scratch, 1, ncclFloat64, ncclSum, static_cast<ncclComm_t>(sh.nccl_comm), ex.side));
  MMSBM_CUDA(cudaEventRecord(signal, ex.side));
  return 0;
}

static int check_shard(const mmsbm_shard_t* sh, const char* who) {
  MMSBM_REQUIRE(sh, MMSBM_EINVAL, "%s: null shard", who);
  MMSBM_REQUIRE(sh->n_users > 0 && sh->n_items > 0 && sh->n_levels > 0 && sh->K > 0 && sh->L > 0 &&
                    sh->n_runs > 0 && sh->n_users_own > 0 && sh->n_items_own > 0 && sh->n_ratings_u >= 0 &&
                    sh->n_ratings_i >= 0, MMSBM_EINVAL, "%s: bad size", who);
  MMSBM_REQUIRE(sh->user_lo >= 0 && sh->user_lo + sh->n_users_own <= sh->n_users && sh->item_lo >= 0 &&
                    sh->item_lo + sh->n_items_own <= sh->n_items, MMSBM_EINVAL, "%s: own range outside the ids", who);
  MMSBM_REQUIRE(sh->world >= 1 && sh->rank >= 0 && sh->rank < sh->world && sh->exchange_dev, MMSBM_EINVAL,
                "%s: bad rank / world / exchange", who);
  for (int r = 0; r < sh->world; ++r)
    MMSBM_REQUIRE(sh->exchange_dev[r], MMSBM_EINVAL, "%s: exchange pointer of rank %d is null", who, r);
  MMSBM_REQUIRE(sh->world == 1 || sh->nccl_comm, MMSBM_EINVAL, "%s: world > 1 needs an NCCL communicator", who);
  MMSBM_REQUIRE(sh->K <= 32 && sh->L <= 32 && sh->n_levels <= 31, MMSBM_ERANGE,
                "%s: sharded runs support K, L <= 32 and R <= 31", who);
  return 0;
}

struct ShardDims {
  int ldk, ldl, rnb_u, rnb_i;
  bool emit_items;
  int64_t pmax_u, pmax_i, lmax_u, lmax_i, smax_u, smax_i;
  size_t p_elems, wg_u, wg_i, partial, slots_u, slots_i, ctr;
};

static ShardDims shard_dims(const mmsbm_shard_t& s) {
  ShardDims d;
  const int S = s.n_runs, R = s.n_levels;
  d.ldk = row_stride(s.K); d.ldl = row_stride(s.L);
  d.rnb_u = R * d.ldl; d.rnb_i = R * d.ldk;
  d.emit_items = s.n_items <= s.n_users;
  d.pmax_u = (int64_t)s.n_users_own + s.n_ratings_u / MMSBM_PIECE_LEN + 1;
  d.pmax_i = (int64_t)s.n_items_own + s.n_ratings_i / MMSBM_PIECE_LEN + 1;
  d.lmax_u = s.n_ratings_u / MMSBM_PIECE_LEN + 1; d.lmax_i = s.n_ratings_i / MMSBM_PIECE_LEN + 1;
  d.smax_u = 2 * (s.n_ratings_u / MMSBM_PIECE_LEN) + 1; d.smax_i = 2 * (s.n_ratings_i / MMSBM_PIECE_LEN) + 1;
  d.p_elems = (size_t)S * d.ldk * d.ldl * R;
  d.wg_u = (size_t)S * s.n_users_own * d.rnb_u;
  d.wg_i = (size_t)S * s.n_items_own * d.rnb_i;
  const size_t pi = (size_t)s.L * R * d.ldk, pu = (size_t)s.K * R * d.ldl;
  d.partial = (size_t)S * kPrSlabs * (pi > pu ? pi : pu);
  d.slots_u = (size_t)S * d.smax_u * d.rnb_u;
  d.slots_i = (size_t)S * d.smax_i * d.rnb_i;
  d.ctr = 2 * ((size_t)S + 8);
  return d;
}

}

using namespace mmsbm;

extern "C" int mmsbm_nccl_load(const char* path) {
  if (g_nccl.handle) return 0;
  void* h = dlopen((path && *path) ? path : "libnccl.so.2", RTLD_NOW | RTLD_GLOBAL);
  MMSBM_REQUIRE(h, MMSBM_ENODEV, "cannot load NCCL (%s): %s", (path && *path) ? path : "libnccl.so.2", dlerror());
  NcclApi api;
  api.handle = h;
  api.GetUniqueId = reinterpret_cast<decltype(api.GetUniqueId)>(dlsym(h, "ncclGetUniqueId"));
  api.CommInitRank = reinterpret_cast<decltype(api.CommInitRank)>(dlsym(h, "ncclCommInitRank"));
  api.CommDestroy = reinterpret_cast<decltype(api.CommDestroy)>(dlsym(h, "ncclCommDestroy"));
  api.AllReduce = reinterpret_cast<decltype(api.AllReduce)>(dlsym(h, "ncclAllReduce"));
  api.GetErrorString = reinterpret_cast<decltype(api.GetErrorString)>(dlsym(h, "ncclGetErrorString"));
  MMSBM_REQUIRE(api.GetUniqueId && api.CommInitRank && api.CommDestroy && api.AllReduce && api.GetErrorString,
                MMSBM_ENODEV, "NCCL library lacks a required symbol");
  g_nccl = api;
  return 0;
}

extern "C" int mmsbm_nccl_unique_id(unsigned char* id128) {
  int rc = nccl_ready();
  if (rc) return rc;
  MMSBM_REQUIRE(id128, MMSBM_EINVAL, "mmsbm_nccl_unique_id: null output");
  static_assert(sizeof(ncclUniqueId) == 128, "ncclUniqueId is 128 bytes");
  ncclUniqueId id;
  MMSBM_NCCL(g_nccl.GetUniqueId(&id));
  memcpy(id128, &id, 128);
  return 0;
}

extern "C" int mmsbm_nccl_comm_init(const unsigned char* id128, int32_t rank, int32_t world, void** comm) {
  int rc = nccl_ready();
  if (rc) return rc;
  MMSBM_REQUIRE(id128 && comm && world >= 1 && rank >= 0 && rank < world, MMSBM_EINVAL,
                "mmsbm_nccl_comm_init: bad argument");
  ncclUniqueId id;
  memcpy(&id, id128, 128);
  ncclComm_t c = nullptr;
  MMSBM_NCCL(g_nccl.CommInitRank(&c, world, id, rank));
  *comm = c;
  return 0;
}

extern "C" int mmsbm_nccl_comm_destroy(void* comm) {
  if (!comm || !g_nccl.handle) return 0;
  MMSBM_NCCL(g_nccl.CommDestroy(static_cast<ncclComm_t>(comm)));
  return 0;
}

extern "C" int mmsbm_ipc_alloc(size_t bytes, void** dev_ptr, unsigned char* handle64) {
  MMSBM_REQUIRE(dev_ptr && handle64 && bytes > 0, MMSBM_EINVAL, "mmsbm_ipc_alloc: bad argument");
  static_assert(sizeof(cudaIpcMemHandle_t) == 64, "cudaIpcMemHandle_t is 64 bytes");
  void* p = nullptr;
  MMSBM_CUDA(cudaMalloc(&p, bytes));
  cudaIpcMemHandle_t h;
  cudaError_t e = cudaIpcGetMemHandle(&h, p);
  if (e != cudaSuccess) {
    cudaFree(p);
    set_error("cudaIpcGetMemHandle failed: %s", cudaGetErrorString(e));
    return (int)e;
  }
  memcpy(handle64, &h, 64);
  *dev_ptr = p;
  return 0;
}
extern "C" int mmsbm_ipc_open(const unsigned char* handle64, void** dev_ptr) {
  MMSBM_REQUIRE(dev_ptr && handle64, MMSBM_EINVAL, "mmsbm_ipc_open: bad argument");
  cudaIpcMemHandle_t h;
  memcpy(&h, handle64, 64);
  MMSBM_CUDA(cudaIpcOpenMemHandle(dev_ptr, h, cudaIpcMemLazyEnablePeerAccess));
  return 0;
}
extern "C" int mmsbm_ipc_close(void* dev_ptr) {
  if (dev_ptr) MMSBM_CUDA(cudaIpcCloseMemHandle(dev_ptr));
  return 0;
}
extern "C" int mmsbm_ipc_free(void* dev_ptr) {
  if (dev_ptr) MMSBM_CUDA(cudaFree(dev_ptr));
  return 0;
}

extern "C" int mmsbm_shard_exchange_bytes(int32_t U, int32_t I, int32_t K, int32_t L, int32_t S, size_t* bytes) {
  MMSBM_REQUIRE(bytes && U > 0 && I > 0 && K > 0 && L > 0 && S > 0, MMSBM_EINVAL,
                "mmsbm_shard_exchange_bytes: bad argument");
  *bytes = grid_layout(U, I, K, L, S).total_bytes;
  return 0;
}

extern "C" int mmsbm_shard_workspace_bytes(const mmsbm_shard_t* sh, size_t* bytes) {
  int rc = check_shard(sh, "mmsbm_shard_workspace_bytes");
  if (rc) return rc;
  MMSBM_REQUIRE(bytes, MMSBM_EINVAL, "mmsbm_shard_workspace_bytes: null output");
  const ShardDims d = shard_dims(*sh);
  *bytes = 4 * align_up(d.p_elems * 8) + align_up(d.wg_u * 8) + align_up(d.wg_i * 8) + align_up(d.partial * 8) +
           align_up(d.slots_u * 8) + align_up(d.slots_i * 8) + align_up(d.ctr * 4) + 256;
  return 0;
}

extern "C" int mmsbm_shard_publish(const mmsbm_shard_t* sh, const double* theta_own, const double* eta_own,
                                   int32_t half, void* stream) {
  int rc = check_shard(sh, "mmsbm_shard_publish");
  if (rc) return rc;
  MMSBM_REQUIRE(theta_own && eta_own && (half == 0 || half == 1), MMSBM_EINVAL, "mmsbm_shard_publish: bad argument");
  if (sh->world > 1 && (rc = nccl_ready())) return rc;
  cudaStream_t st = static_cast<cudaStream_t>(stream);
  const GridLayout g = grid_layout(sh->n_users, sh->n_items, sh->K, sh->L, sh->n_runs);
  Exchange ex;
  if ((rc = ex.open(sh->world))) return rc;
  if (sh->world > 1) {
    MMSBM_CUDA(cudaEventRecord(ex.partial, st));
    MMSBM_CUDA(cudaStreamWaitEvent(ex.side, ex.partial, 0));
  }
  if ((rc = publish_side(*sh, g, g.theta, 2, theta_own, sh->n_users_own, sh->user_lo, half, st, ex))) return rc;
  if ((rc = publish_side(*sh, g, g.eta, 3, eta_own, sh->n_items_own, sh->item_lo, half, st, ex))) return rc;
  if (sh->world > 1) {
    if ((rc = barrier_on_side(*sh, g, ex, ex.arrived[0][0]))) return rc;
    MMSBM_CUDA(cudaStreamWaitEvent(st, ex.arrived[0][0], 0));
  }
  return 0;
}

extern "C" int mmsbm_em_run_sharded(const mmsbm_shard_t* shp, int32_t iterations, double* theta_a, double* eta_a,
                                    double* pr_a, double* theta_b, double* eta_b, double* pr_b, int32_t half,
                                    void* ws, size_t ws_bytes, void* stream, float* prof) {
  int rc = check_shard(shp, "mmsbm_em_run_sharded");
  if (rc) return rc;
  const mmsbm_shard_t& sh = *shp;
  MMSBM_REQUIRE(iterations >= 0 && theta_a && eta_a && pr_a && theta_b && eta_b && pr_b && ws &&
                    (half == 0 || half == 1), MMSBM_EINVAL, "mmsbm_em_run_sharded: bad argument");
  MMSBM_REQUIRE(sh.useg_dev && sh.udeg_dev && sh.usched_dev && sh.iseg_dev && sh.ideg_dev && sh.isched_dev &&
                    (sh.n_ratings_u == 0 || sh.uadj_dev) && (sh.n_ratings_i == 0 || sh.iadj_dev), MMSBM_EINVAL,
                "mmsbm_em_run_sharded: null index pointer");
  const bool peers = sh.world > 1;
  if (peers && (rc = nccl_ready())) return rc;
  cudaStream_t st = static_cast<cudaStream_t>(stream);
  const int S = sh.n_runs, R = sh.n_levels, K = sh.K, L = sh.L;
  const int Uo = sh.n_users_own, Io = sh.n_items_own;
  const ShardDims d = shard_dims(sh);
  const GridLayout g = grid_layout(sh.n_users, sh.n_items, K, L, S);
  Arena arena(ws, ws_bytes);
  double* pw_u = arena.take<double>(d.p_elems);
  double* pn_u = arena.take<double>(d.p_elems);
  double* pw_i = arena.take<double>(d.p_elems);
  double* pn_i = arena.take<double>(d.p_elems);
  double* wg_u = arena.take<double>(d.wg_u);
  double* wg_i = arena.take<double>(d.wg_i);
  double* partial = arena.take<double>(d.partial);
  double* slots_u = arena.take<double>(d.slots_u);
  double* slots_i = arena.take<double>(d.slots_i);
  int32_t* counters = arena.take<int32_t>(d.ctr);
  MMSBM_REQUIRE(pw_u && pn_u && pw_i && pn_i && wg_u && wg_i && partial && slots_u && slots_i && counters,
                MMSBM_ENOMEM, "mmsbm_em_run_sharded: workspace too small (%zu)", ws_bytes);

  Exchange ex;
  if ((rc = ex.open(sh.world))) return rc;
  constexpr int kProf = 7;
  cudaEvent_t ev[kProf] = {nullptr};
  struct Cleanup {
    cudaEvent_t* ev;
    ~Cleanup() {
      for (int k = 0; k < kProf; ++k) if (ev[k]) cudaEventDestroy(ev[k]);
      set_reserved_ctas(0);
    }
  } cleanup{ev};
  if (prof) for (int k = 0; k < kProf; ++k) MMSBM_CUDA(cudaEventCreate(&ev[k]));
  double acc[8] = {0, 0, 0, 0, 0, 0, 0, 0};
#define MMSBM_MARK(k) do { if (prof) MMSBM_CUDA(cudaEventRecord(ev[k], st)); } while (0)

  const int64_t n_big = sh.n_ratings_u > sh.n_ratings_i ? sh.n_ratings_u : sh.n_ratings_i;
  const bool dyn = env_int("MMSBM_DYN", n_big >= ((int64_t)1 << 20) ? 1 : 0) != 0;
  const bool alternate = peers && env_int("MMSBM_SHARD_ALTERNATE", 1) != 0;
  const bool overlap = peers && env_int("MMSBM_SHARD_OVERLAP", 1) != 0;
  const bool fuse = env_int("MMSBM_SHARD_FUSE", 1) != 0;
  if (peers) set_reserved_ctas(env_int("MMSBM_SHARD_RESERVE", 4));
  const void* mine = sh.exchange_dev[sh.rank];
  if (peers) {
    MMSBM_CUDA(cudaEventRecord(ex.partial, st));
    MMSBM_CUDA(cudaStreamWaitEvent(ex.side, ex.partial, 0));
  }
  bool have_arrival[2] = {false, false};

  for (int it = 0; it < iterations; ++it) {
    const bool fwd = (it & 1) == 0;
    const int cur = half ^ (it & 1), nxt = cur ^ 1;
    const double* th = fwd ? theta_a : theta_b; const double* et = fwd ? eta_a : eta_b;
    const double* pr = fwd ? pr_a : pr_b;
    double* th_n = fwd ? theta_b : theta_a; double* et_n = fwd ? eta_b : eta_a; double* pr_n = fwd ? pr_b : pr_a;
    const bool users_first = !alternate || (it & 1) == 0;
    const bool emit_items = d.emit_items;
    const bool emit_after_pass1 = peers && (emit_items != users_first);

    auto pass_users = [&]() -> int {
      if (have_arrival[1]) MMSBM_CUDA(cudaStreamWaitEvent(st, ex.arrived[1][(it + 1) & 1], 0));
      SegArgs a{sh.useg_dev, sh.uadj_dev, sh.usched_dev, table_ptr(mine, g, cur, g.eta[2]), wg_u, slots_u, d.pmax_u,
                d.lmax_u, d.smax_u, Uo, sh.n_items, d.ldl, R, 0, 0, 0, dyn ? counters : nullptr};
      return launch_segment_pass_and_fixup(a, table_ptr(mine, g, cur, g.eta[1]), table_ptr(mine, g, cur, g.eta[0]),
                                           sh.n_ratings_u, S, st);
    };
    auto finish_users = [&](cudaStream_t fs) -> int {
      const RowPublish pub = row_publish(mine, g, g.theta, 2, nxt, sh.n_users, sh.user_lo);
      int r = launch_n(wg_u, pn_u, th, sh.udeg_dev, th_n, Uo, d.ldk, d.rnb_u, 1, S, fs, fuse ? &pub : nullptr);
      if (r) return r;
      return publish_side(sh, g, g.theta, 2, fuse ? nullptr : th_n, Uo, sh.user_lo, nxt, fs, ex);
    };
    auto pass_items = [&]() -> int {
      if (have_arrival[0]) MMSBM_CUDA(cudaStreamWaitEvent(st, ex.arrived[0][(it + 1) & 1], 0));
      SegArgs a{sh.iseg_dev, sh.iadj_dev, sh.isched_dev, table_ptr(mine, g, cur, g.theta[1]), wg_i, slots_i, d.pmax_i,
                d.lmax_i, d.smax_i, Io, sh.n_users, d.ldk, R, 0, 0, 0, dyn ? counters + d.ctr / 2 : nullptr};
      return launch_segment_pass_and_fixup(a, table_ptr(mine, g, cur, g.theta[0]), nullptr, sh.n_ratings_i, S, st);
    };
    auto finish_items = [&](cudaStream_t fs) -> int {
      const RowPublish pub = row_publish(mine, g, g.eta, 3, nxt, sh.n_items, sh.item_lo);
      int r = launch_n(wg_i, pn_i, et, sh.ideg_dev, et_n, Io, d.ldl, d.rnb_i, 1, S, fs, fuse ? &pub : nullptr);
      if (r) return r;
      return publish_side(sh, g, g.eta, 3, fuse ? nullptr : et_n, Io, sh.item_lo, nxt, fs, ex);
    };
    auto reduce_pr = [&](cudaStream_t fs) -> int {
      int r = launch_pr(emit_items ? et : th, emit_items ? wg_i : wg_u, partial, pr, pr_n, emit_items ? Io : Uo,
                        emit_items ? L : K, emit_items ? d.ldl : d.ldk, emit_items ? d.ldk : d.ldl, K, L, R, S,
                        emit_items, !peers, fs);
      if (r || !peers) return r;
      MMSBM_CUDA(cudaEventRecord(ex.partial, fs));
      MMSBM_CUDA(cudaStreamWaitEvent(ex.side, ex.partial, 0));
      MMSBM_NCCL(g_nccl.AllReduce(pr_n, pr_n, (size_t)S * K * L * R, ncclFloat64, ncclSum,
                                  static_cast<ncclComm_t>(sh.nccl_comm), ex.side));
      MMSBM_CUDA(cudaEventRecord(ex.pr_done, ex.side));
      return 0;
    };
    auto after_publish = [&](int which) -> int {
      if (!peers) return 0;
      return barrier_on_side(sh, g, ex, ex.arrived[which][it & 1]);
    };
    cudaStream_t aux = overlap ? ex.aux : st;

    const auto host_t0 = std::chrono::steady_clock::now();
    MMSBM_MARK(0);
    if (dyn) MMSBM_CUDA(cudaMemsetAsync(counters, 0, d.ctr * 4, st));
    if ((rc = launch_prep_p(pr, K, L, R, d.ldk, d.ldl, S, pw_u, pn_u, pw_i, pn_i, st))) return rc;
    if (overlap) {
      MMSBM_CUDA(cudaEventRecord(ex.p_ready, st));
      MMSBM_CUDA(cudaStreamWaitEvent(aux, ex.p_ready, 0));
    }
    if (users_first) {
      if ((rc = launch_w(th, pw_u, wg_u, Uo, d.ldk, d.rnb_u, S, st))) return rc;
      if ((rc = launch_w(et, pw_i, wg_i, Io, d.ldl, d.rnb_i, S, aux))) return rc;
    } else {
      if ((rc = launch_w(et, pw_i, wg_i, Io, d.ldl, d.rnb_i, S, st))) return rc;
      if ((rc = launch_w(th, pw_u, wg_u, Uo, d.ldk, d.rnb_u, S, aux))) return rc;
    }
    if (overlap) MMSBM_CUDA(cudaEventRecord(ex.w2_ready, aux));
    MMSBM_MARK(1);
    if ((rc = users_first ? pass_users() : pass_items())) return rc;
    MMSBM_MARK(2);
    if (overlap) {
      MMSBM_CUDA(cudaEventRecord(ex.pass1_done, st));
      MMSBM_CUDA(cudaStreamWaitEvent(aux, ex.pass1_done, 0));
    }
    if ((rc = users_first ? finish_users(aux) : finish_items(aux))) return rc;
    if (emit_after_pass1 && (rc = reduce_pr(aux))) return rc;
    if ((rc = after_publish(users_first ? 0 : 1))) return rc;
    if (overlap) MMSBM_CUDA(cudaEventRecord(ex.aux_done, aux));
    MMSBM_MARK(3);
    if (overlap) MMSBM_CUDA(cudaStreamWaitEvent(st, ex.w2_ready, 0));
    if ((rc = users_first ? pass_items() : pass_users())) return rc;
    MMSBM_MARK(4);
    if (!emit_after_pass1) {
      if (overlap) {
        MMSBM_CUDA(cudaEventRecord(ex.pass1_done, st));
        MMSBM_CUDA(cudaStreamWaitEvent(aux, ex.pass1_done, 0));
      }
      if ((rc = reduce_pr(aux))) return rc;
      if (overlap) MMSBM_CUDA(cudaEventRecord(ex.aux_done, aux));
    }
    if ((rc = users_first ? finish_items(st) : finish_users(st))) return rc;
    if ((rc = after_publish(users_first ? 1 : 0))) return rc;
    MMSBM_MARK(5);
    if (overlap) MMSBM_CUDA(cudaStreamWaitEvent(st, ex.aux_done, 0));
    if (peers) {
      MMSBM_CUDA(cudaStreamWaitEvent(st, ex.pr_done, 0));
      if ((rc = launch_finalize_pr(pr_n, S * K * L, R, st))) return rc;
      have_arrival[0] = have_arrival[1] = true;
    }
    MMSBM_MARK(6);
    if (prof) {
      acc[7] += std::chrono::duration<double, std::milli>(std::chrono::steady_clock::now() - host_t0).count();
      MMSBM_CUDA(cudaEventSynchronize(ev[6]));
      float t = 0.f;
      cudaEventElapsedTime(&t, ev[0], ev[6]); acc[0] += t;
      cudaEventElapsedTime(&t, ev[5], ev[6]); acc[1] += t;
      for (int k = 0; k < 5; ++k) { cudaEventElapsedTime(&t, ev[k], ev[k + 1]); acc[2 + k] += t; }
    }
  }
#undef MMSBM_MARK
  if (peers && iterations > 0) {
    MMSBM_CUDA(cudaStreamWaitEvent(st, ex.arrived[0][(iterations - 1) & 1], 0));
    MMSBM_CUDA(cudaStreamWaitEvent(st, ex.arrived[1][(iterations - 1) & 1], 0));
  }
  if (prof) for (int k = 0; k < 8; ++k) prof[k] = iterations > 0 ? (float)(acc[k] / iterations) : 0.f;
  return 0;
}
```

Baseline: 26.70 billion.

## Add eight-run octet segment pass with split head/tail interleaved neighbor table

Adds a segment-pass variant that processes eight runs per group, using four lanes that each cover a 16-wide head chunk plus a scalar tail for NB=20. The neighbor table is interleaved in a new layout that puts all runs' heads contiguous and then the tails, and new shuffle reductions (sum4/all4) produce the group normalisation. Run planning, workspace sizing, table publishing and the sharded layout are extended so octets come first, followed by hexas, pairs and singles. The aim is more data reuse per adjacency load and better aligned 256-bit gathers, at the cost of more register pressure and extra code paths.

After: 28.94 billion, median of 6. 1.08x the previous value.

```diff
diff --git a/mmsbm_b200/build.py b/mmsbm_b200/build.py
--- a/mmsbm_b200/build.py
+++ b/mmsbm_b200/build.py
@@ -6,7 +6,7 @@
 HERE = os.path.dirname(os.path.abspath(__file__))
 CSRC = os.path.join(HERE, "csrc")
 LIB = os.path.join(HERE, "libmmsbm_b200.so")
-SOURCES = ["em_step.cu", "em_small.cu", "seg_inst_ch1.cu", "seg_inst_ch2.cu", "seg_inst_ch4.cu", "seg_inst_pair.cu", "seg_inst_hexa.cu", "graph_build.cu",
+SOURCES = ["em_step.cu", "em_small.cu", "seg_inst_ch1.cu", "seg_inst_ch2.cu", "seg_inst_ch4.cu", "seg_inst_pair.cu", "seg_inst_hexa.cu", "seg_inst_octa.cu", "graph_build.cu",
            "reductions.cu", "host_api.cu", "sharded_run.cu", "fold_in.cu"]
 NVCC_FLAGS = [
     "-gencode", "arch=compute_100a,code=sm_100a", "-O3", "-lineinfo", "-std=c++17",
diff --git a/mmsbm_b200/csrc/em_internal.cuh b/mmsbm_b200/csrc/em_internal.cuh
--- a/mmsbm_b200/csrc/em_internal.cuh
+++ b/mmsbm_b200/csrc/em_internal.cuh
@@ -10,8 +10,8 @@
 int sm_count();
 void set_reserved_ctas(int n);
 
-struct RunPlan { int hexas, pairs, pair_group0, single_from; };
-RunPlan plan_runs(int NBp, int n_runs, bool hexa_table);
+struct RunPlan { int octas, hexas, hexa_from, pairs, pair_group0, single_from; };
+RunPlan plan_runs(int NBp, int n_runs, bool wide_groups);
 
 int launch_prep_p(const double* pr, int K, int L, int R, int ldk, int ldl, int n_runs, double* pw_u,
                   double* pn_u, double* pw_i, double* pn_i, cudaStream_t st);
@@ -22,15 +22,15 @@
 int launch_w(const double* own, const double* pw, double* W, int M, int LD, int RNB, int n_runs,
              cudaStream_t st);
 struct RowPublish {
-  double* dst[3];
-  int gs[3], group0[3], groups[3];
+  double* dst[4];
+  int gs[4], run0[4], group0[4], groups[4];
   int n_all, row0;
 };
 int launch_n(const double* G, const double* pn, const double* own, const int32_t* deg, double* out,
              int M, int LD, int RNB, int normalize, int n_runs, cudaStream_t st,
              const RowPublish* publish = nullptr);
 
-int launch_segment_pass_and_fixup(SegArgs a, const double* nbr_pairs, const double* nbr_hexa,
+int launch_segment_pass_and_fixup(SegArgs a, const double* nbr_pairs, const double* nbr_hexa, const double* nbr_octa,
                                   int64_t n_ratings, int n_runs, cudaStream_t st, bool no_long_segments = false);
 
 int launch_pr(const double* own, const double* g, double* partial, const double* pr, double* pr_out,
diff --git a/mmsbm_b200/csrc/em_step.cu b/mmsbm_b200/csrc/em_step.cu
--- a/mmsbm_b200/csrc/em_step.cu
+++ b/mmsbm_b200/csrc/em_step.cu
@@ -42,7 +42,7 @@
   const int id = (int)(rest % n_src);
   const size_t p = group0 + rest / n_src;
   const double4_t v = ldg256(src + (((size_t)(gs * p + j) * n_src + id) * ld + 4 * c));
-  stg256(dst + (((p * n_dst + row0 + id) * gs + j) * ld + 4 * c), v);
+  stg256(dst + (p * n_dst + row0 + id) * gs * ld + gather_offset(gs, ld, j, 4 * c), v);
 }
 
 __global__ void prep_p_kernel(const double* pr, int K, int L, int R, int ldk, int ldl, double* pw_u,
@@ -217,9 +217,10 @@
   int pgs = 1, pj = 0;
   size_t pgrp = 0;
 #pragma unroll
-  for (int t = 0; t < 3; ++t) {
-    if (pub.dst[t] != nullptr && run >= pub.gs[t] * pub.group0[t] && run < pub.gs[t] * (pub.group0[t] + pub.groups[t])) {
-      pdst = pub.dst[t]; pgs = pub.gs[t]; pgrp = (size_t)(run / pub.gs[t]); pj = run % pub.gs[t];
+  for (int t = 0; t < 4; ++t) {
+    const int rr = run - pub.run0[t];
+    if (pub.dst[t] != nullptr && rr >= pub.gs[t] * pub.group0[t] && rr < pub.gs[t] * (pub.group0[t] + pub.groups[t])) {
+      pdst = pub.dst[t]; pgs = pub.gs[t]; pgrp = (size_t)(rr / pub.gs[t]); pj = rr % pub.gs[t];
     }
   }
   {
@@ -281,7 +282,7 @@
         double4_t v{acc[j][4 * c] * ov.x, acc[j][4 * c + 1] * ov.y, acc[j][4 * c + 2] * ov.z, acc[j][4 * c + 3] * ov.w};
         if (normalize) { v.x = v.x / d; v.y = v.y / d; v.z = v.z / d; v.w = v.w / d; }
         stg256(out_run + (size_t)mr[j] * LD + 4 * c, v);
-        if (pdst) stg256(pdst + (((pgrp * pub.n_all + pub.row0 + mr[j]) * pgs + pj) * LD + 4 * c), v);
+        if (pdst) stg256(pdst + (pgrp * pub.n_all + pub.row0 + mr[j]) * pgs * LD + gather_offset(pgs, LD, pj, 4 * c), v);
       }
     }
   }
@@ -483,10 +484,16 @@
   return n_runs >= 6 && NBp == 20 && env_int("MMSBM_HEXA", 1) != 0;
 }
 
-RunPlan plan_runs(int NBp, int n_runs, bool hexa_table) {
-  RunPlan p{0, 0, 0, 0};
-  if (hexa_table && hexa_enabled(NBp, n_runs)) p.hexas = n_runs / 6;
-  p.single_from = 6 * p.hexas;
+static bool octa_enabled(int NBp, int n_runs) {
+  return n_runs >= kOctaRuns && NBp == kOctaNB && env_int("MMSBM_OCTA", 1) != 0;
+}
+
+RunPlan plan_runs(int NBp, int n_runs, bool wide_groups) {
+  RunPlan p{0, 0, 0, 0, 0, 0};
+  if (wide_groups && octa_enabled(NBp, n_runs)) p.octas = n_runs / kOctaRuns;
+  p.hexa_from = kOctaRuns * p.octas;
+  if (wide_groups && hexa_enabled(NBp, n_runs - p.hexa_from)) p.hexas = (n_runs - p.hexa_from) / 6;
+  p.single_from = p.hexa_from + 6 * p.hexas;
   if (pairs_enabled(NBp, n_runs - p.single_from)) {
     p.pairs = (n_runs - p.single_from) / 2;
     p.pair_group0 = p.single_from / 2;
@@ -496,17 +503,37 @@
 }
 
 static int launch_segment_pass_impl(SegArgs a, const double* nbr_pairs, const double* nbr_hexa,
-                                    int64_t n_ratings, int n_runs, cudaStream_t st) {
+                                    const double* nbr_octa, int64_t n_ratings, int n_runs, cudaStream_t st) {
   const double avg_degree = (double)n_ratings / (double)a.nseg;
   PassShape sh = choose_shape(a.NBp, avg_degree);
   const int un_e = env_int("MMSBM_UN", 0), occ_e = env_int("MMSBM_OCC", 0);
-  const RunPlan plan = plan_runs(a.NBp, n_runs, nbr_hexa != nullptr);
+  const RunPlan plan = plan_runs(a.NBp, n_runs, nbr_hexa != nullptr || nbr_octa != nullptr);
   const int single_from = plan.single_from;
+  if (plan.octas > 0) {
+    MMSBM_REQUIRE(nbr_octa, MMSBM_EINVAL, "segment pass: the table of run octets is missing");
+    const int octas = plan.octas;
+    SegArgs p = a;
+    p.nbr = nbr_octa;
+    p.run_base = 0;
+    p.grp_base = 0;
+    p.segs_per_cta = segs_per_cta_for(a.pmax, n_ratings, octas);
+    const unsigned gx = grid_x_for(p, 3);
+    if (p.counters) a.counters += octas;
+    const size_t smem = seg_smem_bytes(p, kOctaRuns);
+    MMSBM_REQUIRE(smem <= 227 * 1024, MMSBM_ERANGE, "segment pass needs %zu bytes of shared memory", smem);
+    const int rc = launch_segment_pass_octa(p, 4, 3, 3, dim3(gx, octas), smem, st);
+    if (rc) {
+      if (rc == MMSBM_ERANGE) set_error("no eight-run segment-pass variant");
+      return rc;
+    }
+    if (single_from == n_runs && plan.pairs == 0 && plan.hexas == 0) return 0;
+  }
   if (plan.hexas > 0) {
+    MMSBM_REQUIRE(nbr_hexa, MMSBM_EINVAL, "segment pass: the table of six-run groups is missing");
     const int hexas = plan.hexas;
     SegArgs p = a;
     p.nbr = nbr_hexa;
-    p.run_base = 0;
+    p.run_base = plan.hexa_from;
     p.grp_base = 0;
     p.segs_per_cta = segs_per_cta_for(a.pmax, n_ratings, hexas);
     const unsigned gx = grid_x_for(p, occ_e > 0 ? occ_e : 3);
@@ -528,7 +555,7 @@
     const int pairs = plan.pairs;
     SegArgs p = a;
     p.nbr = nbr_pairs;
-    p.run_base = 6 * plan.hexas;
+    p.run_base = 2 * plan.pair_group0;
     p.grp_base = plan.pair_group0;
     p.counters = a.counters;
     p.segs_per_cta = segs_per_cta_for(a.pmax, n_ratings, pairs);
@@ -575,9 +602,9 @@
   return rc;
 }
 
-int launch_segment_pass_and_fixup(SegArgs a, const double* nbr_pairs, const double* nbr_hexa,
+int launch_segment_pass_and_fixup(SegArgs a, const double* nbr_pairs, const double* nbr_hexa, const double* nbr_octa,
                                   int64_t n_ratings, int n_runs, cudaStream_t st, bool no_long_segments) {
-  int rc = launch_segment_pass_impl(a, nbr_pairs, nbr_hexa, n_ratings, n_runs, st);
+  int rc = launch_segment_pass_impl(a, nbr_pairs, nbr_hexa, nbr_octa, n_ratings, n_runs, st);
   if (rc) return rc;
   if (no_long_segments) return 0;
   const int64_t fix_ctas = 4 * sm_count();
@@ -723,8 +750,10 @@
   bool emit_items;
   int nseg_e, NA_e, NBp_e;
   size_t p_elems, wg_u_elems, wg_i_elems, partial_elems, slots_u_elems, slots_i_elems;
+  RunPlan plan_u, plan_i;
   size_t th2_elems, et2_elems;
   size_t et6_elems;
+  size_t et8_elems;
   size_t ctr_elems;
   int64_t lmax, smax, pmax_u, pmax_i;
 };
@@ -748,9 +777,12 @@
   d.pmax_i = (int64_t)I + N / MMSBM_PIECE_LEN + 1;
   d.slots_u_elems = (size_t)S * d.smax * d.rnb_u;
   d.slots_i_elems = (size_t)S * d.smax * d.rnb_i;
-  d.th2_elems = (size_t)(S / 2) * 2 * U * d.ldk;
-  d.et2_elems = (size_t)(S / 2) * 2 * I * d.ldl;
-  d.et6_elems = (size_t)(S / 6) * 6 * I * d.ldl;
+  d.plan_u = plan_runs(d.ldl, S, true);
+  d.plan_i = plan_runs(d.ldk, S, false);
+  d.th2_elems = (size_t)(d.plan_i.pair_group0 + d.plan_i.pairs) * 2 * U * d.ldk;
+  d.et2_elems = (size_t)(d.plan_u.pair_group0 + d.plan_u.pairs) * 2 * I * d.ldl;
+  d.et6_elems = (size_t)d.plan_u.hexas * 6 * I * d.ldl;
+  d.et8_elems = (size_t)d.plan_u.octas * kOctaRuns * I * d.ldl;
   d.ctr_elems = 2 * ((size_t)S + 8);
   return d;
 }
@@ -758,7 +790,8 @@
 static size_t em_main_bytes(const EmDims& d) {
   return 4 * align_up(d.p_elems * 8) + align_up(d.wg_u_elems * 8) + align_up(d.wg_i_elems * 8) +
          align_up(d.partial_elems * 8) + align_up(d.slots_u_elems * 8) + align_up(d.slots_i_elems * 8) +
-         align_up(d.th2_elems * 8) + align_up(d.et2_elems * 8) + align_up(d.et6_elems * 8) + align_up(d.ctr_elems * 4) + 256;
+         align_up(d.th2_elems * 8) + align_up(d.et2_elems * 8) + align_up(d.et6_elems * 8) + align_up(d.et8_elems * 8) +
+         align_up(d.ctr_elems * 4) + 256;
 }
 
 }
@@ -810,12 +843,21 @@
   double* th2 = arena.take<double>(d.th2_elems);
   double* et2 = arena.take<double>(d.et2_elems);
   double* et6 = arena.take<double>(d.et6_elems);
+  double* et8 = arena.take<double>(d.et8_elems);
   int32_t* counters = arena.take<int32_t>(d.ctr_elems);
-  MMSBM_REQUIRE(pw_u && pn_u && pw_i && pn_i && wg_u && wg_i && partial && slots_u && slots_i && th2 && et2 && et6 && counters,
+  MMSBM_REQUIRE(pw_u && pn_u && pw_i && pn_i && wg_u && wg_i && partial && slots_u && slots_i && th2 && et2 && et6 && et8 &&
+                    counters,
                 MMSBM_ENOMEM,
                 "mmsbm_em_step: workspace too small (%zu)", ws_bytes);
   int rc;
   const bool dyn = env_int("MMSBM_DYN", N >= ((int64_t)1 << 22) ? 1 : 0) != 0;
+  auto interleave_user_tables = [&](cudaStream_t s) {
+    const RunPlan& pu = d.plan_u;
+    int r = launch_interleave(eta, et8, I, I, 0, d.ldl, 0, pu.octas, kOctaRuns, s);
+    if (!r) r = launch_interleave(eta + (size_t)pu.hexa_from * I * d.ldl, et6, I, I, 0, d.ldl, 0, pu.hexas, 6, s);
+    if (!r) r = launch_interleave(eta, et2, I, I, 0, d.ldl, pu.pair_group0, pu.pairs, 2, s);
+    return r;
+  };
 #define MMSBM_MARK(k) do { if (ev) MMSBM_CUDA(cudaEventRecord(ev[k], st)); } while (0)
   MMSBM_MARK(0);
   cudaStream_t s2 = ov ? ov->side : st;
@@ -833,23 +875,22 @@
                        d.NA_e, d.emit_items ? d.ldl : d.ldk, d.NBp_e, K, L, R, S, d.emit_items,
                        (flags & MMSBM_RAW_ETA_PR) == 0, s);
     };
-    if (hexa_enabled(d.ldl, S) && (rc = launch_interleave(eta, et6, I, I, 0, d.ldl, 0, S / 6, 6, st))) return rc;
-    if (pairs_enabled(d.ldl, S) && (rc = launch_interleave(eta, et2, I, I, 0, d.ldl, 0, S / 2, 2, st))) return rc;
+    if ((rc = interleave_user_tables(st))) return rc;
     if ((rc = launch_w(theta, pw_u, wg_u, U, d.ldk, d.rnb_u, S, st))) return rc;
     {
       SegArgs a{useg, uadj, usched, eta, wg_u, slots_u, d.pmax_u, d.lmax, d.smax, U, I, d.ldl, R, 0, 0, 0,
                 dyn ? counters : nullptr};
-      if ((rc = launch_segment_pass_and_fixup(a, et2, et6, N, S, st, ov->no_long_u))) return rc;
+      if ((rc = launch_segment_pass_and_fixup(a, et2, et6, et8, N, S, st, ov->no_long_u))) return rc;
     }
     if ((rc = launch_n(wg_u, pn_u, theta, udeg, theta_out, U, d.ldk, d.rnb_u,
                        (flags & MMSBM_RAW_THETA) ? 0 : 1, S, st))) return rc;
     if (!d.emit_items && (rc = pr_step(st))) return rc;
-    if (pairs_enabled(d.ldk, S) && (rc = launch_interleave(theta, th2, U, U, 0, d.ldk, 0, S / 2, 2, s2))) return rc;
+    if ((rc = launch_interleave(theta, th2, U, U, 0, d.ldk, d.plan_i.pair_group0, d.plan_i.pairs, 2, s2))) return rc;
     if ((rc = launch_w(eta, pw_i, wg_i, I, d.ldl, d.rnb_i, S, s2))) return rc;
     {
       SegArgs a{iseg, iadj, isched, theta, wg_i, slots_i, d.pmax_i, d.lmax, d.smax, I, U, d.ldk, R, 0, 0, 0,
                 dyn ? counters + d.ctr_elems / 2 : nullptr};
-      if ((rc = launch_segment_pass_and_fixup(a, th2, nullptr, N, S, s2, ov->no_long_i))) return rc;
+      if ((rc = launch_segment_pass_and_fixup(a, th2, nullptr, nullptr, N, S, s2, ov->no_long_i))) return rc;
     }
     if ((rc = launch_n(wg_i, pn_i, eta, ideg, eta_out, I, d.ldl, d.rnb_i,
                        (flags & MMSBM_RAW_ETA_PR) ? 0 : 1, S, s2))) return rc;
@@ -861,9 +902,8 @@
     if (dyn) MMSBM_CUDA(cudaMemsetAsync(counters, 0, d.ctr_elems * 4, st));
     if ((rc = launch_prep_p(pr, K, L, R, d.ldk, d.ldl, S, pw_u, pn_u, pw_i, pn_i, st))) return rc;
     MMSBM_FORK(0);
-    if (hexa_enabled(d.ldl, S) && (rc = launch_interleave(eta, et6, I, I, 0, d.ldl, 0, S / 6, 6, st))) return rc;
-    if (pairs_enabled(d.ldl, S) && (rc = launch_interleave(eta, et2, I, I, 0, d.ldl, 0, S / 2, 2, st))) return rc;
-    if (pairs_enabled(d.ldk, S) && (rc = launch_interleave(theta, th2, U, U, 0, d.ldk, 0, S / 2, 2, st))) return rc;
+    if ((rc = interleave_user_tables(st))) return rc;
+    if ((rc = launch_interleave(theta, th2, U, U, 0, d.ldk, d.plan_i.pair_group0, d.plan_i.pairs, 2, st))) return rc;
     if ((rc = launch_w(theta, pw_u, wg_u, U, d.ldk, d.rnb_u, S, st))) return rc;
     if ((rc = launch_w(eta, pw_i, wg_i, I, d.ldl, d.rnb_i, S, s2))) return rc;
     MMSBM_SIDE_DONE(1);
@@ -872,7 +912,7 @@
   {
     SegArgs a{useg, uadj, usched, eta, wg_u, slots_u, d.pmax_u, d.lmax, d.smax, U, I, d.ldl, R, 0, 0, 0,
               dyn ? counters : nullptr};
-    if ((rc = launch_segment_pass_and_fixup(a, et2, et6, N, S, st, ov && ov->no_long_u))) return rc;
+    if ((rc = launch_segment_pass_and_fixup(a, et2, et6, et8, N, S, st, ov && ov->no_long_u))) return rc;
   }
   MMSBM_MARK(2);
   MMSBM_FORK(2);
@@ -884,7 +924,7 @@
   {
     SegArgs a{iseg, iadj, isched, theta, wg_i, slots_i, d.pmax_i, d.lmax, d.smax, I, U, d.ldk, R, 0, 0, 0,
               dyn ? counters + d.ctr_elems / 2 : nullptr};
-    if ((rc = launch_segment_pass_and_fixup(a, th2, nullptr, N, S, st, ov && ov->no_long_i))) return rc;
+    if ((rc = launch_segment_pass_and_fixup(a, th2, nullptr, nullptr, N, S, st, ov && ov->no_long_i))) return rc;
   }
   MMSBM_MARK(4);
   MMSBM_FORK(3);
diff --git a/mmsbm_b200/csrc/seg_inst_octa.cu b/mmsbm_b200/csrc/seg_inst_octa.cu
--- /dev/null
+++ b/mmsbm_b200/csrc/seg_inst_octa.cu
@@ -0,0 +1,7 @@
+#include "segment_pass.cuh"
+namespace mmsbm {
+int launch_segment_pass_octa(const SegArgs& a, int G, int UN, int MINB, dim3 grid, size_t smem, cudaStream_t st) {
+  MMSBM_SEG_LAUNCH_R(4, 1, 3, 3, 8)
+  return MMSBM_ERANGE;
+}
+}
diff --git a/mmsbm_b200/csrc/segment_pass.cuh b/mmsbm_b200/csrc/segment_pass.cuh
--- a/mmsbm_b200/csrc/segment_pass.cuh
+++ b/mmsbm_b200/csrc/segment_pass.cuh
@@ -39,6 +39,13 @@
   const double e = fma(-x, r, 1.0);
   const double t = fma(e, e, e);
   return fma(r, t, r);
+}
+
+constexpr int kOctaRuns = 8, kOctaNB = 20, kOctaHead = 16;
+__host__ __device__ constexpr int gather_offset(int gs, int ld, int j, int b) {
+  return gs != kOctaRuns ? j * ld + b
+         : b < kOctaHead ? j * kOctaHead + b
+                         : kOctaRuns * kOctaHead + j * (kOctaNB - kOctaHead) + (b - kOctaHead);
 }
 
 struct SegArgs {
@@ -88,6 +95,21 @@
     u += is3 ? 0.0 : x2;
     const double x3 = __shfl_sync(kFull, u, r3);
     return (is1 ? v : u) + x3;
+  }
+  __device__ __forceinline__ double sum4(double a0, double a1, double a2, double a3) const {
+    static_assert(G == 4, "sum4 is the 4-lane schedule");
+    const double t0 = (is1 | is3 ? a1 : a0) + __shfl_xor_sync(kFull, is1 | is3 ? a0 : a1, 1);
+    const double t1 = (is1 | is3 ? a3 : a2) + __shfl_xor_sync(kFull, is1 | is3 ? a2 : a3, 1);
+    return (is2 | is3 ? t1 : t0) + __shfl_xor_sync(kFull, is2 | is3 ? t0 : t1, 2);
+  }
+  __device__ __forceinline__ void all4(double v, double out[4]) const {
+    static_assert(G == 4, "all4 is the 4-lane schedule");
+    const double p2 = __shfl_xor_sync(kFull, v, 2);
+    const double lo = (is2 | is3) ? p2 : v, hi = (is2 | is3) ? v : p2;
+    const double plo = __shfl_xor_sync(kFull, lo, 1), phi = __shfl_xor_sync(kFull, hi, 1);
+    const bool odd = is1 | is3;
+    out[0] = odd ? plo : lo; out[1] = odd ? lo : plo;
+    out[2] = odd ? phi : hi; out[3] = odd ? hi : phi;
   }
   __device__ __forceinline__ double from_lane(double x, int j) const { return __shfl_sync(kFull, x, lead + j); }
   __device__ __forceinline__ double operator()(double p) const {
@@ -126,13 +148,15 @@
 template <int G, int CH, int UN, int MINB, int RUNS>
 __global__ void __launch_bounds__(kWarps * 32, MINB)
 segment_pass_kernel(const SegArgs A) {
+  constexpr bool OCTA = RUNS == kOctaRuns;
+  static_assert(!OCTA || (G == 4 && CH == 1), "an octet is 4 lanes x (one 256-bit + one 64-bit piece) per run");
   constexpr int GR = G * RUNS;
   constexpr int RPS = 32 / GR;
   constexpr int SLOTS = UN * RPS;
   static_assert(SLOTS <= 32, "a chunk's ids must fit one coalesced 32-lane load");
   extern __shared__ __align__(32) unsigned char smem_raw[];
   const int lane = threadIdx.x & 31, warp = threadIdx.x >> 5;
-  const int R = A.R, NBp = (CH == 1) ? 4 * G : A.NBp, RNB = R * NBp;
+  const int R = A.R, NBp = OCTA ? kOctaNB : (CH == 1) ? 4 * G : A.NBp, RNB = R * NBp;
   const int NCH = NBp >> 2;
 
   constexpr int WB = w_buffers(RUNS);
@@ -156,6 +180,7 @@
   const int first = dyn ? blockIdx.x * kWarps + warp : seg_lo + warp;
   const int claim_base = dyn ? gridDim.x * kWarps : seg_lo + kWarps;
   const double* nbr_run = (RUNS == 1) ? A.nbr + (size_t)run * A.nnbr * NBp
+                          : OCTA      ? A.nbr + (size_t)(A.grp_base + blockIdx.y) * A.nnbr * RUNS * NBp
                                       : A.nbr + ((size_t)(A.grp_base + blockIdx.y) * A.nnbr * RUNS + rsel) * NBp;
   int coff[CH];
   bool con[CH];
@@ -165,6 +190,7 @@
     con[c] = lane_on && chunk < NCH;
     coff[c] = con[c] ? 4 * chunk : 0;
   }
+  const int hoff = gather_offset(RUNS, NBp, rsel, 4 * q), toff = gather_offset(RUNS, NBp, rsel, kOctaHead + q);
   const GroupSum<G> group_sum(grp * GR + rsel * G, q);
 
   auto fetch_w = [&](int s_, int b_) {
@@ -217,7 +243,9 @@
                               : A.partial + ((size_t)run * A.smax + slot) * RNB;
 
     double4_t g[CH], wr[CH];
+    double gt = 0.0, wt = 0.0;
     auto flush = [&](int r, bool any) {
+      if constexpr (OCTA) gout[r * NBp + kOctaHead + q] = gt;
 #pragma unroll
       for (int c = 0; c < CH; ++c) {
         double4_t v = g[c];
@@ -242,16 +270,19 @@
       const int le = min(end, __shfl_sync(kFull, bend_reg, r + 1));
 #pragma unroll
       for (int c = 0; c < CH; ++c) g[c] = double4_t{0.0, 0.0, 0.0, 0.0};
+      gt = 0.0;
       const bool any = lo < le;
       if (any) {
 #pragma unroll
         for (int c = 0; c < CH; ++c)
           wr[c] = con[c] ? lds32(wb + r * NBp + coff[c]) : double4_t{0.0, 0.0, 0.0, 0.0};
+        if constexpr (OCTA) wt = wb[r * NBp + kOctaHead + q];
         for (int base = lo; base < le; base += SLOTS) {
           const int cnt = min(SLOTS, le - base);
           auto chunk = [&](auto ns_tag) {
             constexpr int NS = decltype(ns_tag)::value;
             double4_t x[NS][CH];
+            [[maybe_unused]] double xt[NS];
 #pragma unroll
             for (int un = 0; un < NS; ++un) {
               const int sl = un * RPS + grp;
@@ -259,8 +290,13 @@
               if (sl >= cnt) id = 0;
               MMSBM_DEV_CHECK(id >= 0 && id < A.nnbr);
               const double* row = nbr_run + (size_t)id * (RUNS * NBp);
-#pragma unroll
-              for (int c = 0; c < CH; ++c) x[un][c] = ldg256(row + coff[c]);
+              if constexpr (OCTA) {
+                x[un][0] = ldg256(row + hoff);
+                xt[un] = __ldg(row + toff);
+              } else {
+#pragma unroll
+                for (int c = 0; c < CH; ++c) x[un][c] = ldg256(row + coff[c]);
+              }
             }
             {
               const int nxt = base + cnt + lane;
@@ -275,9 +311,15 @@
                 part = fma(x[un][c].x, wr[c].x, part); part2 = fma(x[un][c].y, wr[c].y, part2);
                 part = fma(x[un][c].z, wr[c].z, part); part2 = fma(x[un][c].w, wr[c].w, part2);
               }
+              if constexpr (OCTA) part = fma(xt[un], wt, part);
               im[un] = part + part2;
             }
-            if constexpr (G == 5 && NS == 3) {
+            if constexpr (OCTA && NS >= 3) {
+              double all[4];
+              group_sum.all4(rcp_clamped(group_sum.sum4(im[0], im[1], im[2], NS == 4 ? im[NS - 1] : 0.0)), all);
+#pragma unroll
+              for (int un = 0; un < NS; ++un) im[un] = all[un];
+            } else if constexpr (G == 5 && NS == 3) {
               const double mine = rcp_clamped(group_sum.sum3(im[0], im[1], im[2]));
 #pragma unroll
               for (int un = 0; un < NS; ++un) {
@@ -298,6 +340,7 @@
                 g[c].x = fma(x[un][c].x, im[un], g[c].x); g[c].y = fma(x[un][c].y, im[un], g[c].y);
                 g[c].z = fma(x[un][c].z, im[un], g[c].z); g[c].w = fma(x[un][c].w, im[un], g[c].w);
               }
+              if constexpr (OCTA) gt = fma(xt[un], im[un], gt);
             }
           };
           static_assert(UN <= 6, "extend the step-count dispatch");
@@ -324,6 +367,7 @@
 int launch_segment_pass_ch1(const SegArgs& a, int G, int UN, int MINB, dim3 grid, size_t smem, cudaStream_t st);
 int launch_segment_pass_pair(const SegArgs& a, int G, int UN, int MINB, dim3 grid, size_t smem, cudaStream_t st);
 int launch_segment_pass_hexa(const SegArgs& a, int G, int UN, int MINB, dim3 grid, size_t smem, cudaStream_t st);
+int launch_segment_pass_octa(const SegArgs& a, int G, int UN, int MINB, dim3 grid, size_t smem, cudaStream_t st);
 int launch_segment_pass_ch2(const SegArgs& a, int G, int UN, int MINB, dim3 grid, size_t smem, cudaStream_t st);
 int launch_segment_pass_ch4(const SegArgs& a, int G, int UN, int MINB, dim3 grid, size_t smem, cudaStream_t st);
 int launch_segment_pass_ch8(const SegArgs& a, int G, int UN, int MINB, dim3 grid, size_t smem, cudaStream_t st);
diff --git a/mmsbm_b200/csrc/sharded_run.cu b/mmsbm_b200/csrc/sharded_run.cu
--- a/mmsbm_b200/csrc/sharded_run.cu
+++ b/mmsbm_b200/csrc/sharded_run.cu
@@ -34,9 +34,9 @@
   return 0;
 }
 
-struct Table { size_t off; int gs, group0, groups, ld, n_all; };
+struct Table { size_t off; int gs, run0, group0, groups, ld, n_all; };
 struct GridLayout {
-  Table eta[3], theta[2];
+  Table eta[4], theta[2];
   size_t half_bytes, total_bytes;
 };
 
@@ -45,15 +45,16 @@
   const RunPlan pu = plan_runs(ldl, S, true), pi = plan_runs(ldk, S, false);
   GridLayout g{};
   size_t off = 0;
-  auto put = [&](Table& t, int gs, int group0, int groups, int ld, int n_all, int addr_groups) {
-    t = Table{off, gs, group0, groups, ld, n_all};
+  auto put = [&](Table& t, int gs, int run0, int group0, int groups, int ld, int n_all, int addr_groups) {
+    t = Table{off, gs, run0, group0, groups, ld, n_all};
     off += align_up((size_t)addr_groups * gs * n_all * ld * 8);
   };
-  put(g.eta[0], 6, 0, pu.hexas, ldl, I, pu.hexas);
-  put(g.eta[1], 2, pu.pair_group0, pu.pairs, ldl, I, pu.pairs ? S / 2 : 0);
-  put(g.eta[2], 1, pu.single_from, S - pu.single_from, ldl, I, S > pu.single_from ? S : 0);
-  put(g.theta[0], 2, pi.pair_group0, pi.pairs, ldk, U, pi.pairs ? S / 2 : 0);
-  put(g.theta[1], 1, pi.single_from, S - pi.single_from, ldk, U, S > pi.single_from ? S : 0);
+  put(g.eta[0], kOctaRuns, 0, 0, pu.octas, ldl, I, pu.octas);
+  put(g.eta[1], 6, pu.hexa_from, 0, pu.hexas, ldl, I, pu.hexas);
+  put(g.eta[2], 2, 0, pu.pair_group0, pu.pairs, ldl, I, pu.pairs ? S / 2 : 0);
+  put(g.eta[3], 1, 0, pu.single_from, S - pu.single_from, ldl, I, S > pu.single_from ? S : 0);
+  put(g.theta[0], 2, 0, pi.pair_group0, pi.pairs, ldk, U, pi.pairs ? S / 2 : 0);
+  put(g.theta[1], 1, 0, pi.single_from, S - pi.single_from, ldk, U, S > pi.single_from ? S : 0);
   g.half_bytes = off;
   g.total_bytes = 2 * off + 256;
   return g;
@@ -62,12 +63,12 @@
 static RowPublish row_publish(const void* base, const GridLayout& g, const Table* tabs, int n_tabs, int half,
                               int n_all, int row0) {
   RowPublish p{};
-  for (int k = 0; k < n_tabs && k < 3; ++k) {
+  for (int k = 0; k < n_tabs && k < 4; ++k) {
     const Table& t = tabs[k];
     if (t.groups == 0) continue;
     p.dst[k] = reinterpret_cast<double*>(const_cast<char*>(static_cast<const char*>(base)) +
                                          (size_t)half * g.half_bytes + t.off);
-    p.gs[k] = t.gs; p.group0[k] = t.group0; p.groups[k] = t.groups;
+    p.gs[k] = t.gs; p.run0[k] = t.run0; p.group0[k] = t.group0; p.groups[k] = t.groups;
   }
   p.n_all = n_all; p.row0 = row0;
   return p;
@@ -128,7 +129,8 @@
     const Table& t = tabs[k];
     if (t.groups == 0) continue;
     double* dst = reinterpret_cast<double*>(mine + (size_t)half * g.half_bytes + t.off);
-    int rc = launch_interleave(own_rows, dst, n_own, t.n_all, lo, t.ld, t.group0, t.groups, t.gs, st);
+    int rc = launch_interleave(own_rows + (size_t)t.run0 * n_own * t.ld, dst, n_own, t.n_all, lo, t.ld, t.group0,
+                               t.groups, t.gs, st);
     if (rc) return rc;
   }
   if (sh.world == 1) return 0;
@@ -320,7 +322,7 @@
     MMSBM_CUDA(cudaStreamWaitEvent(ex.side, ex.partial, 0));
   }
   if ((rc = publish_side(*sh, g, g.theta, 2, theta_own, sh->n_users_own, sh->user_lo, half, st, ex))) return rc;
-  if ((rc = publish_side(*sh, g, g.eta, 3, eta_own, sh->n_items_own, sh->item_lo, half, st, ex))) return rc;
+  if ((rc = publish_side(*sh, g, g.eta, 4, eta_own, sh->n_items_own, sh->item_lo, half, st, ex))) return rc;
   if (sh->world > 1) {
     if ((rc = barrier_on_side(*sh, g, ex, ex.arrived[0][0]))) return rc;
     MMSBM_CUDA(cudaStreamWaitEvent(st, ex.arrived[0][0], 0));
@@ -400,10 +402,10 @@
 
     auto pass_users = [&]() -> int {
       if (have_arrival[1]) MMSBM_CUDA(cudaStreamWaitEvent(st, ex.arrived[1][(it + 1) & 1], 0));
-      SegArgs a{sh.useg_dev, sh.uadj_dev, sh.usched_dev, table_ptr(mine, g, cur, g.eta[2]), wg_u, slots_u, d.pmax_u,
+      SegArgs a{sh.useg_dev, sh.uadj_dev, sh.usched_dev, table_ptr(mine, g, cur, g.eta[3]), wg_u, slots_u, d.pmax_u,
                 d.lmax_u, d.smax_u, Uo, sh.n_items, d.ldl, R, 0, 0, 0, dyn ? counters : nullptr};
-      return launch_segment_pass_and_fixup(a, table_ptr(mine, g, cur, g.eta[1]), table_ptr(mine, g, cur, g.eta[0]),
-                                           sh.n_ratings_u, S, st);
+      return launch_segment_pass_and_fixup(a, table_ptr(mine, g, cur, g.eta[2]), table_ptr(mine, g, cur, g.eta[1]),
+                                           table_ptr(mine, g, cur, g.eta[0]), sh.n_ratings_u, S, st);
     };
     auto finish_users = [&](cudaStream_t fs) -> int {
       const RowPublish pub = row_publish(mine, g, g.theta, 2, nxt, sh.n_users, sh.user_lo);
@@ -415,13 +417,13 @@
       if (have_arrival[0]) MMSBM_CUDA(cudaStreamWaitEvent(st, ex.arrived[0][(it + 1) & 1], 0));
       SegArgs a{sh.iseg_dev, sh.iadj_dev, sh.isched_dev, table_ptr(mine, g, cur, g.theta[1]), wg_i, slots_i, d.pmax_i,
                 d.lmax_i, d.smax_i, Io, sh.n_users, d.ldk, R, 0, 0, 0, dyn ? counters + d.ctr / 2 : nullptr};
-      return launch_segment_pass_and_fixup(a, table_ptr(mine, g, cur, g.theta[0]), nullptr, sh.n_ratings_i, S, st);
+      return launch_segment_pass_and_fixup(a, table_ptr(mine, g, cur, g.theta[0]), nullptr, nullptr, sh.n_ratings_i, S, st);
     };
     auto finish_items = [&](cudaStream_t fs) -> int {
-      const RowPublish pub = row_publish(mine, g, g.eta, 3, nxt, sh.n_items, sh.item_lo);
+      const RowPublish pub = row_publish(mine, g, g.eta, 4, nxt, sh.n_items, sh.item_lo);
       int r = launch_n(wg_i, pn_i, et, sh.ideg_dev, et_n, Io, d.ldl, d.rnb_i, 1, S, fs, fuse ? &pub : nullptr);
       if (r) return r;
-      return publish_side(sh, g, g.eta, 3, fuse ? nullptr : et_n, Io, sh.item_lo, nxt, fs, ex);
+      return publish_side(sh, g, g.eta, 4, fuse ? nullptr : et_n, Io, sh.item_lo, nxt, fs, ex);
     };
     auto reduce_pr = [&](cudaStream_t fs) -> int {
       int r = launch_pr(emit_items ? et : th, emit_items ? wg_i : wg_u, partial, pr, pr_n, emit_items ? Io : Uo,
```
